# RchalYang/torchrl

Hardware: NVIDIA H100
Metric: env_steps_per_sec (higher is better)
Workload: dtype f32

## Files before the change

### include/torchrl_b200.h

```cpp
#ifndef TORCHRL_B200_H
#define TORCHRL_B200_H
#include <stdint.h>

#ifdef __cplusplus
extern "C" {
#endif

#define TRL_OK 0
#define TRL_EINVAL (-1)
#define TRL_EALIGN (-2)
#define TRL_EUNSUPPORTED (-3)

const char* trl_last_error(void);
int trl_abi_version(void);
int trl_device_info(int* sm_count, int* cc_major, int* cc_minor);

int trl_gae_scan(const float* rewards, const float* values, const uint8_t* terminals,
                 const uint8_t* time_limits, const float* last_value, float* advs, float* returns,
                 int64_t T, int64_t N, float gamma, float tau, int time_limit_filter, int variant,
                 void* stream);

int trl_discount_return(const float* rewards, const float* values, const uint8_t* terminals,
                        const uint8_t* time_limits, const float* last_value, float* advs, float* returns,
                        int64_t T, int64_t N, float gamma, int time_limit_filter, int variant,
                        void* stream);

int trl_synth_env_smem_bytes(int obs_dim, int act_dim);
int trl_synth_env_num_ctas(int64_t N);
int trl_synth_env_step(float* state, const float* actions, const float* A, const float* B, const float* c,
                       const float* lb, const float* ub, int* elapsed, const int* step_count, float* reward,
                       uint8_t* done, uint8_t* time_limit, double* partial, double* batch_sums,
                       double* norm_mean, double* norm_var, double* norm_count, unsigned* ticket,
                       int* any_reset, const int* t_ptr, int64_t N, int obs_dim, int act_dim, float rho,
                       float eta, float ctrl_cost, float term_thr, float reward_scale, int max_episode_steps,
                       int max_episode_frames, int merge_stats, void* stream);
int trl_synth_env_reset(float* state, int* elapsed, unsigned* episode, const unsigned* seeds,
                        const uint8_t* mask, int64_t N, int obs_dim, double init_scale, void* stream);
int trl_synth_env_seed(unsigned* seeds, unsigned* episode, int64_t N, unsigned seed, unsigned n_total,
                       unsigned first_env, void* stream);

int trl_obs_norm_moments(const float* x, int64_t N, int obs_dim, double* sums, void* stream);
int trl_obs_norm_merge(const double* sums, double batch_n, int obs_dim, double* mean, double* var,
                       double* count, void* stream);
int trl_obs_norm_filt(const float* raw, const double* mean, const double* var, int64_t N, int obs_dim,
                      double clip, float* out, void* stream);

int trl_tanh_gaussian_sample(const float* mean, const float* log_std, int ls_stride, const float* eps,
                             float noise_scale, uint64_t seed, const uint64_t* rng_counter, int64_t M,
                             int act_dim, int tanh_action, float* action, float* pre_tanh, float* log_prob,
                             float* eps_out, int* nan_flag, void* stream);
int trl_tanh_gaussian_sample_bwd(const float* action, const float* eps, const float* log_std, int ls_stride,
                                 const float* g_action, const float* g_logp, int64_t M, int act_dim,
                                 int tanh_action, float* g_mean, float* g_log_std, void* stream);

int trl_collect_finalize(const float* cur_ob_in, const float* next_norm, float* state, const float* act,
                         const float* value, const float* v_next, const float* reward, const uint8_t* done,
                         const uint8_t* tl, int* elapsed, unsigned* episode, const unsigned* seeds,
                         int* step_count, double* ep_return, double* epoch_reward, float* ret_log,
                         int* n_done, const int* any_reset, const double* norm_mean, const double* norm_var,
                         float* cur_ob_out, float* b_obs, float* b_next_obs, float* b_acts, float* b_values,
                         float* b_rewards, uint8_t* b_terminals, uint8_t* b_time_limits, const int* t_ptr,
                         int64_t N, int obs_dim, int act_dim, int max_episode_frames, float discount,
                         double init_scale, double clip, int terminal_includes_surpass,
                         int raw_obs_after_reset, void* stream);
int trl_step_advance(int* t_ptr, int T, int* size_ptr, uint64_t* rng_counter, void* stream);

int trl_row_gather(int nkeys, const void* const* src, void* const* dst, const int64_t* row_bytes,
                   const int64_t* idx, const int* pos_ptr, int rows, void* stream);
int trl_ring_write(int nkeys, const void* const* src, void* const* dst, const int64_t* row_bytes,
                   const int* row_ptr, void* stream);
int trl_ring_write_advance(int nkeys, const void* const* src, void* const* dst, const int64_t* row_bytes,
                           int* row_ptr, int T, int* size_ptr, unsigned* ticket, void* stream);
int trl_vec_stats(const float* x, int64_t n, float* stats4, void* stream);
int trl_vec_moments(const float* x, int64_t n, double* moments4, void* stream);
int trl_row_group_moments(const float* x, const int64_t* idx, int groups, int b, int64_t row_elems,
                          double* moments4, void* stream);
int trl_group_stats_from_moments(const double* gathered, int world, int groups, double n_total, float* stats4,
                                 void* stream);
int trl_vec_stats_from_moments(const double* gathered, int world, double n_total, float* stats4, void* stream);

int64_t trl_ppo_actor_scratch_doubles(int64_t B, int act_dim);
int trl_ppo_actor_loss(const float* mean, const float* log_std, int ls_stride, const float* actions,
                       const float* old_logp, const float* advs, const float* adv_stats,
                       const int* adv_stats_pos ,
                       int64_t B,
                       int act_dim, int tanh_action, float clip_para, float entropy_coeff, float ls_min, float ls_max,
                       float* g_mean, float* g_log_std, float* logp_out, float* info16, double* scratch, unsigned* ticket,
                       void* stream);
int trl_ppo_critic_loss(const float* values, const float* returns, const float* old_values, int64_t B,
                        int clipped, float clip_para, float* g_values, float* info1, double* scratch,
                        unsigned* ticket, void* stream);
int trl_gaussian_log_prob(const float* mean, const float* log_std, int ls_stride, const float* actions,
                          int64_t B, int act_dim, int tanh_action, float* logp, void* stream);

int trl_categorical_sample(const float* logits, const float* u, uint64_t seed, const uint64_t* rng_counter, int64_t M,
                           int num_actions, float* action, float* log_prob, int* nan_flag, void* stream);
int trl_categorical_log_prob(const float* logits, const float* actions, int64_t M, int num_actions, float* logp,
                             void* stream);
int64_t trl_ppo_categorical_actor_scratch_doubles(int64_t B);
int trl_ppo_categorical_actor_loss(const float* logits, const float* actions, const float* old_logp, const float* advs,
                                   const float* adv_stats, const int* adv_stats_pos, int64_t B, int num_actions,
                                   float clip_para, float entropy_coeff, float* g_logits, float* logp_out,
                                   float* info16, double* scratch, unsigned* ticket, void* stream);

int trl_grad_sumsq_blocks(int nseg);
int trl_grad_sumsq(const float* grad, const int64_t* seg_begin_host, int nseg, unsigned active_mask,
                   double* sumsq3_out, int* step_counts, double beta1, double beta2, double* scratch,
                   unsigned* ticket, void* stream);
int trl_adam_step(float* param, float* grad, float* exp_avg, float* exp_avg_sq, const int64_t* seg_begin_host,
                  int nseg, unsigned active_mask, const double* sumsq3, const float* lr_dev,
                  const float* max_norm_host, const float* eps_host, float beta1, float beta2,
                  float grad_scale, int zero_grad, float* param_hi, float* param_lo, void* stream);
int trl_polyak_update(float* target, const float* source, int64_t n, float tau, float* target_hi,
                      float* target_lo, void* stream);

int64_t trl_offpolicy_scratch_doubles(int64_t B);
int trl_td_target(const float* rewards, const uint8_t* terminals, const float* q1_next, const float* q2_next,
                  const float* logp_next, const float* log_alpha, float fixed_alpha, float gamma, int64_t B,
                  float* y, float* info1, double* scratch, unsigned* ticket, void* stream);
int trl_td3_smooth_action(const float* action, const float* eps, float sigma, float noise_clip, uint64_t seed,
                          const uint64_t* rng_counter, int64_t n, float* out, void* stream);
int trl_sac_alpha_step(const float* logp, float target_entropy, float* log_alpha, float* adam_state3, float lr,
                       float beta1, float beta2, float eps, int64_t B, float* info2, double* scratch,
                       unsigned* ticket, void* stream);
int trl_sac_policy_loss(const float* logp, const float* q1, const float* q2, const float* log_alpha,
                        float fixed_alpha, int64_t B, float* g_logp, float* g_q1, float* g_q2, float* info5,
                        double* scratch, unsigned* ticket, void* stream);
int trl_twin_mse_loss(const float* q1, const float* q2, const float* y, int64_t B, float* g1, float* g2,
                      float* info2, double* scratch, unsigned* ticket, void* stream);
int trl_qr_dqn_loss(const float* pred, const float* next, const float* actions, const float* rewards,
                    const uint8_t* terminals, const float* weights, int B, int n_actions, int n_quantiles,
                    float gamma, float kappa, int mse, float* grad, float* td_out, float* info3, double* scratch,
                    unsigned* ticket, void* stream);

int64_t trl_bias_act_bwd_scratch_floats(int64_t M, int H);
int trl_bias_act_fwd(float* z, const float* bias, int64_t M, int H, int act, void* stream);
int trl_bias_act_bwd(const float* grad, const float* out, float* grad_pre, float* dbias, int64_t M, int H,
                     int act, float* scratch, unsigned* tickets, void* stream);
int trl_split_tf32(const float* x, int64_t n, float* hi, float* lo, void* stream);

int trl_per_sample(const float* prio, int size, const double* u, int b, float beta, int64_t* idx,
                   float* weights, void* stream);
int trl_per_update(float* prio, const int64_t* idx, const float* td, int b, int n, float alpha, float eps,
                   float* max_prio, void* stream);
int trl_per_insert(float* prio, const int* row_ptr, const float* max_prio, void* stream);

int trl_frame_ring_write(const uint8_t* stack, uint8_t* ring, uint8_t* age_ring, const int* elapsed, uint8_t* hist,
                         int* hist_count, const int* top, const int* size, int64_t N, int C, int64_t F, int T, int frame,
                         void* stream);
int trl_frame_hist_advance(int* hist_count, const int* size, int T, void* stream);
int trl_frame_stack_gather(const uint8_t* obs_last, const uint8_t* next_last, const uint8_t* age, const uint8_t* hist,
                           const int* hist_count, const int64_t* idx, const int* pos, int rows, const int* top,
                           const int* size, int64_t N, int C, int64_t F, int T, float scale, float* out_obs,
                           float* out_next, void* stream);

int trl_comm_flag_bytes(void);
int trl_comm_ipc_handle_bytes(void);
int trl_comm_alloc(int64_t bytes, void** ptr_out);
int trl_comm_free(void* ptr);
int trl_comm_ipc_get(void* ptr, void* handle_out);
int trl_comm_ipc_open(const void* handle, void** ptr_out);
int trl_comm_ipc_close(void* ptr);
int trl_comm_scratch_doubles(int nseg);
int trl_allreduce_grad(const void* const* peer_data, void* const* peer_flags, int rank, int world, float* out,
                       int64_t n, const int64_t* seg_begin_host, int nseg, unsigned active_mask, double* sumsq3_out,
                       int* step_counts, double beta1, double beta2, double* scratch, unsigned* ticket, unsigned* seq,
                       int zero_local, void* stream);
int trl_allreduce_f64(const void* const* peer_data, void* const* peer_flags, int rank, int world, double* out, int n,
                      int gather, unsigned* seq, void* stream);
int64_t trl_comm_ll_recv_bytes(int world, int nmax);
int trl_allreduce_f64_ll(const double* local, void* const* peer_recv, int rank, int world, double* out, int n, int nmax,
                         int gather, unsigned* ll_seq, void* stream);

int trl_gemm_tf32x3_nt(const float* A, const float* B, float* C, int64_t M, int64_t K, int splits,
                       float* workspace, const float* bias, int act, void* stream);
int trl_gemm_tf32x3_tn(const float* A, const float* B, float* C, int64_t M, int64_t K, int splits,
                       float* workspace, void* stream);
int trl_transpose_f32(const float* in, float* out, int64_t rows, int cols, void* stream);
int trl_gemm3_pair(const float* A, const float* b_hi, const float* b_lo, float* C, int64_t M, int64_t K,
                   int b_nmajor, const float* bias, int act, void* stream);
int trl_gemm3_pair_tn(const float* A, const float* B, float* C, int64_t M, int64_t K, int splits,
                      float* workspace, void* stream);
int trl_gemm3_pair_tn_cluster(const float* A, const float* B, float* C, int64_t M, int64_t K, int splits,
                              float* workspace, int* tickets, void* stream);

int trl_skinny_k_fwd(const float* X, const float* W, const float* bias, float* Y, int64_t M, int K, int H,
                     int act, void* stream);
int64_t trl_skinny_tn_scratch_floats(int64_t M, int H, int K);
int trl_skinny_tn(const float* A, const float* B, float* Out, float* colsum, int64_t M, int H, int K,
                  int out_transposed, float* scratch, void* stream);
int trl_skinny_n_fwd(const float* X, const float* W, const float* bias, float* Y, int64_t M, int H, int N,
                     void* stream);
int trl_skinny_n_dgrad(const float* G, const float* W, float* dX, int64_t M, int H, int N, void* stream);
int trl_skinny_act_wgrad(const float* G, const float* Y, const float* X, float* dW, float* db, int64_t M, int H,
                         int K, int act, float* scratch, void* stream);
int64_t trl_skinny_dgrad_act_scratch_floats(int64_t M, int H);
int trl_skinny_n_dgrad_act(const float* G, const float* W, const float* Y, float* gz, float* db, int64_t M, int H,
                           int N, int act, float* scratch, void* stream);
int trl_skinny_tn_partial(const float* A, const float* B, int64_t M, int H, int K, int want_colsum, float* scratch,
                          void* stream);
int trl_skinny_act_wgrad_partial(const float* G, const float* Y, const float* X, int64_t M, int H, int K, int act,
                                 float* scratch, void* stream);
int trl_skinny_n_dgrad_act_partial(const float* G, const float* W, const float* Y, float* gz, int64_t M, int H, int N,
                                   int act, float* scratch, void* stream);
int trl_skinny_reduce_jobs(int njobs, const int* kind, const float* const* scratch, float* const* out,
                           float* const* colsum, const int64_t* M, const int* H, const int* K, const int* out_transposed,
                           void* stream);

int trl_synth_atari_step(uint8_t* obs, int* latent, const float* actions, int* elapsed, float* reward,
                         uint8_t* done, uint8_t* time_limit, int64_t N, int max_steps, void* stream);
int trl_synth_atari_reset(uint8_t* obs, int* latent, int* elapsed, unsigned* episode, const unsigned* seeds,
                          const uint8_t* mask, const int* zero_is_mask, int episode_bias, int bump, int64_t N,
                          void* stream);
int trl_u8_to_f32(const uint8_t* in, float* out, int64_t n, float scale, void* stream);

#ifdef __cplusplus
}
#endif
#endif
```

### torchrl_b200/_lib.py

```python
import ctypes
import os

_HERE = os.path.dirname(os.path.abspath(__file__))
LIB_PATH = os.path.join(_HERE, "lib", "libtorchrl_b200.so")

c_f32p = ctypes.c_void_p
c_u8p = ctypes.c_void_p
c_i32p = ctypes.c_void_p
c_i64p = ctypes.c_void_p
c_f64p = ctypes.c_void_p
vp = ctypes.c_void_p
i64 = ctypes.c_int64
i32 = ctypes.c_int
f32 = ctypes.c_float
f64 = ctypes.c_double
u64 = ctypes.c_uint64
u32 = ctypes.c_uint32

SIGNATURES = {
    "trl_last_error": [],
    "trl_abi_version": [],
    "trl_device_info": [vp, vp, vp],
    "trl_gae_scan": [vp, vp, vp, vp, vp, vp, vp, i64, i64, f32, f32, i32, i32, vp],
    "trl_discount_return": [vp, vp, vp, vp, vp, vp, vp, i64, i64, f32, i32, i32, vp],
    "trl_synth_env_smem_bytes": [i32, i32],
    "trl_synth_env_num_ctas": [i64],
    "trl_synth_env_step": [vp] * 20 + [i64, i32, i32, f32, f32, f32, f32, f32, i32, i32, i32, vp],
    "trl_synth_env_reset": [vp, vp, vp, vp, vp, i64, i32, f64, vp],
    "trl_synth_env_seed": [vp, vp, i64, u32, u32, u32, vp],
    "trl_obs_norm_moments": [vp, i64, i32, vp, vp],
    "trl_obs_norm_merge": [vp, f64, i32, vp, vp, vp, vp],
    "trl_obs_norm_filt": [vp, vp, vp, i64, i32, f64, vp, vp],
    "trl_tanh_gaussian_sample": [vp, vp, i32, vp, f32, u64, vp, i64, i32, i32, vp, vp, vp, vp, vp, vp],
    "trl_tanh_gaussian_sample_bwd": [vp, vp, vp, i32, vp, vp, i64, i32, i32, vp, vp, vp],
    "trl_collect_finalize": [vp] * 29 + [i64, i32, i32, i32, f32, f64, f64, i32, i32, vp],
    "trl_step_advance": [vp, i32, vp, vp, vp],
    "trl_row_gather": [i32, vp, vp, vp, vp, vp, i32, vp],
    "trl_ring_write": [i32, vp, vp, vp, vp, vp],
    "trl_ring_write_advance": [i32, vp, vp, vp, vp, i32, vp, vp, vp],
    "trl_vec_stats": [vp, i64, vp, vp],
    "trl_vec_moments": [vp, i64, vp, vp],
    "trl_vec_stats_from_moments": [vp, i32, f64, vp, vp],
    "trl_row_group_moments": [vp, vp, i32, i32, i64, vp, vp],
    "trl_group_stats_from_moments": [vp, i32, i32, f64, vp, vp],
    "trl_ppo_actor_scratch_doubles": [i64, i32],
    "trl_ppo_actor_loss": [vp, vp, i32, vp, vp, vp, vp, vp, i64, i32, i32, f32, f32, f32, f32, vp, vp, vp, vp, vp, vp, vp],
    "trl_ppo_critic_loss": [vp, vp, vp, i64, i32, f32, vp, vp, vp, vp, vp],
    "trl_gaussian_log_prob": [vp, vp, i32, vp, i64, i32, i32, vp, vp],
    "trl_categorical_sample": [vp, vp, u64, vp, i64, i32, vp, vp, vp, vp],
    "trl_categorical_log_prob": [vp, vp, i64, i32, vp, vp],
    "trl_ppo_categorical_actor_scratch_doubles": [i64],
    "trl_ppo_categorical_actor_loss": [vp, vp, vp, vp, vp, vp, i64, i32, f32, f32, vp, vp, vp, vp, vp, vp],
    "trl_grad_sumsq_blocks": [i32],
    "trl_grad_sumsq": [vp, vp, i32, u32, vp, vp, f64, f64, vp, vp, vp],
    "trl_adam_step": [vp, vp, vp, vp, vp, i32, u32, vp, vp, vp, vp, f32, f32, f32, i32, vp, vp, vp],
    "trl_polyak_update": [vp, vp, i64, f32, vp, vp, vp],
    "trl_bias_act_bwd_scratch_floats": [i64, i32],
    "trl_bias_act_fwd": [vp, vp, i64, i32, i32, vp],
    "trl_split_tf32": [vp, i64, vp, vp, vp],
    "trl_bias_act_bwd": [vp, vp, vp, vp, i64, i32, i32, vp, vp, vp],
    "trl_per_sample": [vp, i32, vp, i32, f32, vp, vp, vp],
    "trl_per_update": [vp, vp, vp, i32, i32, f32, f32, vp, vp],
    "trl_per_insert": [vp, vp, vp, vp],
    "trl_gemm_tf32x3_nt": [vp, vp, vp, i64, i64, i32, vp, vp, i32, vp],
    "trl_gemm_tf32x3_tn": [vp, vp, vp, i64, i64, i32, vp, vp],
    "trl_transpose_f32": [vp, vp, i64, i32, vp],
    "trl_frame_ring_write": [vp, vp, vp, vp, vp, vp, vp, vp, i64, i32, i64, i32, i32, vp],
    "trl_frame_hist_advance": [vp, vp, i32, vp],
    "trl_frame_stack_gather": [vp, vp, vp, vp, vp, vp, vp, i32, vp, vp, i64, i32, i64, i32, f32, vp, vp, vp],
    "trl_comm_flag_bytes": [],
    "trl_comm_ipc_handle_bytes": [],
    "trl_comm_alloc": [i64, vp],
    "trl_comm_free": [vp],
    "trl_comm_ipc_get": [vp, vp],
    "trl_comm_ipc_open": [vp, vp],
    "trl_comm_ipc_close": [vp],
    "trl_comm_scratch_doubles": [i32],
    "trl_allreduce_grad": [vp, vp, i32, i32, vp, i64, vp, i32, u32, vp, vp, f64, f64, vp, vp, vp, i32, vp],
    "trl_allreduce_f64": [vp, vp, i32, i32, vp, i32, i32, vp, vp],
    "trl_comm_ll_recv_bytes": [i32, i32],
    "trl_allreduce_f64_ll": [vp, vp, i32, i32, vp, i32, i32, i32, vp, vp],
    "trl_gemm3_pair": [vp, vp, vp, vp, i64, i64, i32, vp, i32, vp],
    "trl_gemm3_pair_tn": [vp, vp, vp, i64, i64, i32, vp, vp],
    "trl_gemm3_pair_tn_cluster": [vp, vp, vp, i64, i64, i32, vp, vp, vp],
    "trl_skinny_k_fwd": [vp, vp, vp, vp, i64, i32, i32, i32, vp],
    "trl_skinny_tn_scratch_floats": [i64, i32, i32],
    "trl_skinny_tn": [vp, vp, vp, vp, i64, i32, i32, i32, vp, vp],
    "trl_skinny_n_fwd": [vp, vp, vp, vp, i64, i32, i32, vp],
    "trl_skinny_n_dgrad": [vp, vp, vp, i64, i32, i32, vp],
    "trl_skinny_act_wgrad": [vp, vp, vp, vp, vp, i64, i32, i32, i32, vp, vp],
    "trl_skinny_dgrad_act_scratch_floats": [i64, i32],
    "trl_skinny_n_dgrad_act": [vp, vp, vp, vp, vp, i64, i32, i32, i32, vp, vp],
    "trl_skinny_tn_partial": [vp, vp, i64, i32, i32, i32, vp, vp],
    "trl_skinny_act_wgrad_partial": [vp, vp, vp, i64, i32, i32, i32, vp, vp],
    "trl_skinny_n_dgrad_act_partial": [vp, vp, vp, vp, i64, i32, i32, i32, vp, vp],
    "trl_skinny_reduce_jobs": [i32, vp, vp, vp, vp, vp, vp, vp, vp, vp],
    "trl_synth_atari_step": [vp, vp, vp, vp, vp, vp, vp, i64, i32, vp],
    "trl_synth_atari_reset": [vp, vp, vp, vp, vp, vp, vp, i32, i32, i64, vp],
    "trl_u8_to_f32": [vp, vp, i64, f32, vp],
    "trl_offpolicy_scratch_doubles": [i64],
    "trl_td_target": [vp, vp, vp, vp, vp, vp, f32, f32, i64, vp, vp, vp, vp, vp],
    "trl_td3_smooth_action": [vp, vp, f32, f32, u64, vp, i64, vp, vp],
    "trl_sac_alpha_step": [vp, f32, vp, vp, f32, f32, f32, f32, i64, vp, vp, vp, vp],
    "trl_sac_policy_loss": [vp, vp, vp, vp, f32, i64, vp, vp, vp, vp, vp, vp, vp],
    "trl_twin_mse_loss": [vp, vp, vp, i64, vp, vp, vp, vp, vp, vp],
    "trl_qr_dqn_loss": [vp, vp, vp, vp, vp, vp, i32, i32, i32, f32, f32, i32, vp, vp, vp, vp, vp, vp],
}
_RESTYPES = {"trl_last_error": ctypes.c_char_p, "trl_ppo_actor_scratch_doubles": ctypes.c_int64,
             "trl_ppo_categorical_actor_scratch_doubles": ctypes.c_int64,
             "trl_offpolicy_scratch_doubles": ctypes.c_int64, "trl_bias_act_bwd_scratch_floats": ctypes.c_int64,
             "trl_skinny_tn_scratch_floats": ctypes.c_int64,
             "trl_skinny_dgrad_act_scratch_floats": ctypes.c_int64, "trl_comm_ll_recv_bytes": ctypes.c_int64}
_VALUE_FUNCS = ("trl_abi_version", "trl_synth_env_smem_bytes", "trl_synth_env_num_ctas", "trl_comm_flag_bytes",
                "trl_comm_ipc_handle_bytes", "trl_comm_scratch_doubles", "trl_comm_ll_recv_bytes",
                "trl_ppo_actor_scratch_doubles", "trl_ppo_categorical_actor_scratch_doubles", "trl_grad_sumsq_blocks")

_lib = None


class NativeLibraryError(RuntimeError):
    pass


def load():
    global _lib
    if _lib is not None:
        return _lib
    if not os.path.exists(LIB_PATH) and os.environ.get("TORCHRL_B200_NO_AUTOBUILD") != "1":
        try:
            from . import build as _build
            _build.build()
        except Exception as e:
            raise NativeLibraryError("%s not found and the in-tree nvcc build failed (%s); there is no CPU "
                                     "fallback" % (LIB_PATH, e)) from e
    if not os.path.exists(LIB_PATH):
        raise NativeLibraryError(
            "%s not found: build it with `python -m torchrl_b200.build` (there is no CPU fallback)" % LIB_PATH)
    lib = ctypes.CDLL(LIB_PATH)
    for name, argtypes in SIGNATURES.items():
        try:
            fn = getattr(lib, name)
        except AttributeError as e:
            raise NativeLibraryError("symbol %s missing from %s" % (name, LIB_PATH)) from e
        fn.argtypes = argtypes
        fn.restype = _RESTYPES.get(name, ctypes.c_int)
    _lib = lib
    return lib


def check(rc, name):
    if rc != 0:
        msg = load().trl_last_error()
        raise RuntimeError("%s failed (rc=%d): %s" % (name, rc, msg.decode() if msg else ""))


_LAUNCHES = 0


def launch_count():
    return _LAUNCHES


def add_launches(n):
    global _LAUNCHES
    _LAUNCHES += int(n)


def call(name, *args):
    global _LAUNCHES
    lib = load()
    rc = getattr(lib, name)(*args)
    if rc != 0:
        check(rc, name)
    _LAUNCHES += 1
```

### torchrl_b200/csrc/gemm_wgmma.cuh

```cuda
#pragma once
#include "common.cuh"
#include "reduce.cuh"
#include <cuda.h>

namespace trl {
namespace wg {

constexpr int kBM = 128, kBN = 128, kN = 256, kBK = 32;
constexpr int kTileBytes = 128 * kBK * 4;
constexpr int kConsumers = 256;
constexpr int kThreads = kConsumers + 128;
constexpr int kProducerRegs = 40, kConsumerRegs = 232;

template <bool BMN, bool BSPLIT>
struct Ring {
  static constexpr int kTiles = 3 + (BMN ? (BSPLIT ? 2 : 1) : 0);
  static constexpr int kStageBytes = kTiles * kTileBytes;
  static constexpr int kStages = (200 * 1024) / kStageBytes < 4 ? (200 * 1024) / kStageBytes : 4;
  static constexpr int kSmemBytes = kStages * kStageBytes + 1024  + 128 ;
  static constexpr bool kConvertB = BMN || !BSPLIT;
  static_assert(kStages >= 2 && kSmemBytes <= 227 * 1024, "fits one sm_90 CTA");
};

__device__ __forceinline__ uint32_t smem_u32(const void* p) { return static_cast<uint32_t>(__cvta_generic_to_shared(p)); }
__device__ __forceinline__ void mbar_init(uint64_t* bar, uint32_t count) {
  asm volatile("mbarrier.init.shared::cta.b64 [%0], %1;" ::"r"(smem_u32(bar)), "r"(count));
}
__device__ __forceinline__ void mbar_arrive(uint64_t* bar) {
  asm volatile("mbarrier.arrive.shared::cta.b64 _, [%0];" ::"r"(smem_u32(bar)) : "memory");
}
__device__ __forceinline__ void mbar_arrive_expect_tx(uint64_t* bar, uint32_t bytes) {
  asm volatile("mbarrier.arrive.expect_tx.shared::cta.b64 _, [%0], %1;" ::"r"(smem_u32(bar)), "r"(bytes) : "memory");
}
__device__ __forceinline__ void mbar_wait(uint64_t* bar, uint32_t parity) {
  uint32_t done;
  do {
    asm volatile(
        "{\n\t"
        ".reg .pred p;\n\t"
        "mbarrier.try_wait.parity.shared::cta.b64 p, [%1], %2;\n\t"
        "selp.u32 %0, 1, 0, p;\n\t"
        "}"
        : "=r"(done)
        : "r"(smem_u32(bar)), "r"(parity)
        : "memory");
  } while (!done);
}
__device__ __forceinline__ void tma_load_2d(void* smem_dst, const CUtensorMap* map, uint64_t* bar, int c_inner, int c_outer) {
  asm volatile(
      "cp.async.bulk.tensor.2d.shared::cluster.global.mbarrier::complete_tx::bytes [%0], [%1, {%3, %4}], [%2];" ::"r"(
          smem_u32(smem_dst)),
      "l"(reinterpret_cast<uint64_t>(map)), "r"(smem_u32(bar)), "r"(c_inner), "r"(c_outer)
      : "memory");
}

__device__ __forceinline__ uint64_t desc_k_sw128(uint32_t smem_addr) {
  uint64_t d = 0;
  d |= static_cast<uint64_t>((smem_addr >> 4) & 0x3FFF);
  d |= static_cast<uint64_t>(1) << 16;
  d |= static_cast<uint64_t>(1024 >> 4) << 32;
  d |= static_cast<uint64_t>(1) << 62;
  return d;
}

__device__ __forceinline__ void wgmma_m64n128k8_tf32_rs(float (&d)[64], const uint32_t (&a)[4], uint64_t desc_b) {
  asm volatile(
      "{\n\t"
      ".reg .pred p;\n\t"
      "setp.ne.b32 p, %69, 0;\n\t"
      "wgmma.mma_async.sync.aligned.m64n128k8.f32.tf32.tf32 "
      "{%0, %1, %2, %3, %4, %5, %6, %7, %8, %9, %10, %11, %12, %13, %14, %15, "
      "%16, %17, %18, %19, %20, %21, %22, %23, %24, %25, %26, %27, %28, %29, %30, %31, "
      "%32, %33, %34, %35, %36, %37, %38, %39, %40, %41, %42, %43, %44, %45, %46, %47, "
      "%48, %49, %50, %51, %52, %53, %54, %55, %56, %57, %58, %59, %60, %61, %62, %63}, "
      "{%64, %65, %66, %67}, %68, p, 1, 1;\n\t"
      "}"
      : "+f"(d[0]), "+f"(d[1]), "+f"(d[2]), "+f"(d[3]), "+f"(d[4]), "+f"(d[5]), "+f"(d[6]), "+f"(d[7]),
        "+f"(d[8]), "+f"(d[9]), "+f"(d[10]), "+f"(d[11]), "+f"(d[12]), "+f"(d[13]), "+f"(d[14]), "+f"(d[15]),
        "+f"(d[16]), "+f"(d[17]), "+f"(d[18]), "+f"(d[19]), "+f"(d[20]), "+f"(d[21]), "+f"(d[22]), "+f"(d[23]),
        "+f"(d[24]), "+f"(d[25]), "+f"(d[26]), "+f"(d[27]), "+f"(d[28]), "+f"(d[29]), "+f"(d[30]), "+f"(d[31]),
        "+f"(d[32]), "+f"(d[33]), "+f"(d[34]), "+f"(d[35]), "+f"(d[36]), "+f"(d[37]), "+f"(d[38]), "+f"(d[39]),
        "+f"(d[40]), "+f"(d[41]), "+f"(d[42]), "+f"(d[43]), "+f"(d[44]), "+f"(d[45]), "+f"(d[46]), "+f"(d[47]),
        "+f"(d[48]), "+f"(d[49]), "+f"(d[50]), "+f"(d[51]), "+f"(d[52]), "+f"(d[53]), "+f"(d[54]), "+f"(d[55]),
        "+f"(d[56]), "+f"(d[57]), "+f"(d[58]), "+f"(d[59]), "+f"(d[60]), "+f"(d[61]), "+f"(d[62]), "+f"(d[63])
      : "r"(a[0]), "r"(a[1]), "r"(a[2]), "r"(a[3]), "l"(desc_b), "r"(1));
}

__device__ __forceinline__ float4 lds128(uint32_t addr) {
  float4 v;
  asm volatile("ld.shared.v4.f32 {%0, %1, %2, %3}, [%4];" : "=f"(v.x), "=f"(v.y), "=f"(v.z), "=f"(v.w) : "r"(addr));
  return v;
}
__device__ __forceinline__ float lds32(uint32_t addr) {
  float v;
  asm volatile("ld.shared.f32 %0, [%1];" : "=f"(v) : "r"(addr));
  return v;
}
__device__ __forceinline__ void sts128(uint32_t addr, const float4 v) {
  asm volatile("st.shared.v4.f32 [%0], {%1, %2, %3, %4};" ::"r"(addr), "f"(v.x), "f"(v.y), "f"(v.z), "f"(v.w));
}
__device__ __forceinline__ uint32_t cluster_rank() {
  uint32_t r;
  asm volatile("mov.u32 %0, %%cluster_ctarank;" : "=r"(r));
  return r;
}
__device__ __forceinline__ uint32_t cluster_size() {
  uint32_t n;
  asm volatile("mov.u32 %0, %%cluster_nctarank;" : "=r"(n));
  return n;
}
__device__ __forceinline__ void cluster_arrive() { asm volatile("barrier.cluster.arrive.release;" ::: "memory"); }
__device__ __forceinline__ void cluster_wait() { asm volatile("barrier.cluster.wait.acquire;" ::: "memory"); }
__device__ __forceinline__ float4 ld_cluster128(uint32_t addr, uint32_t rank) {
  uint32_t remote;
  asm volatile("mapa.shared::cluster.u32 %0, %1, %2;" : "=r"(remote) : "r"(addr), "r"(rank));
  float4 v;
  asm volatile("ld.shared::cluster.v4.f32 {%0, %1, %2, %3}, [%4];"
               : "=f"(v.x), "=f"(v.y), "=f"(v.z), "=f"(v.w)
               : "r"(remote)
               : "memory");
  return v;
}
__device__ __forceinline__ uint32_t tf32_bits(float x) {
  uint32_t u;
  asm("cvt.rna.tf32.f32 %0, %1;" : "=r"(u) : "f"(x));
  return u;
}
__device__ __forceinline__ float4 tf32_hi(const float4 v) {
  return make_float4(__uint_as_float(tf32_bits(v.x)), __uint_as_float(tf32_bits(v.y)), __uint_as_float(tf32_bits(v.z)),
                     __uint_as_float(tf32_bits(v.w)));
}
__device__ __forceinline__ float4 sub4(const float4 a, const float4 b) {
  return make_float4(a.x - b.x, a.y - b.y, a.z - b.z, a.w - b.w);
}

__device__ __forceinline__ float4 load_unit_mn(uint32_t raw, int u, int& row, int& chunk) {
  row = u & 127; chunk = u >> 7;
  const uint32_t a = raw + static_cast<uint32_t>(chunk * 4 * 128 + row) * 4u;
  return make_float4(lds32(a), lds32(a + 512u), lds32(a + 1024u), lds32(a + 1536u));
}
__device__ __forceinline__ uint32_t sw128(int row, int chunk) {
  return static_cast<uint32_t>(row * 128 + ((chunk ^ (row & 7)) << 4));
}

template <bool AMN>
__device__ __forceinline__ uint32_t a_offset(int m, int k) {
  if (!AMN) return static_cast<uint32_t>(m * 128 + ((((k >> 2) ^ (m & 7))) << 4) + (k & 3) * 4);
  return static_cast<uint32_t>((m >> 5) * 4096 + k * 128 + ((((m & 31) >> 2) ^ (k & 7)) << 4) + (m & 3) * 4);
}

struct Params {
  const float* __restrict__ bias;
  int act;
  float* __restrict__ C;
  long long M;
  int k_blocks_per_split;
  float* __restrict__ ws;
  unsigned* tickets;
};

constexpr int kTileLd = kBN + 8;

template <bool AMN, bool BMN, bool BSPLIT, bool TANH_MUFU, bool CLUSTER = false>
__global__ void __launch_bounds__(kThreads, 1)
gemm3_wgmma_kernel(const __grid_constant__ CUtensorMap map_a, const __grid_constant__ CUtensorMap map_b,
                   const __grid_constant__ CUtensorMap map_b2, const Params p) {
  using R = Ring<BMN, BSPLIT>;
  constexpr int S = R::kStages;
  constexpr int kA = 0, kBhi = kTileBytes, kBlo = 2 * kTileBytes, kBraw = 3 * kTileBytes, kBraw2 = 4 * kTileBytes;
  extern __shared__ uint8_t smem_raw[];
  uint8_t* ring = reinterpret_cast<uint8_t*>((reinterpret_cast<uintptr_t>(smem_raw) + 1023) & ~static_cast<uintptr_t>(1023));
  uint64_t* bars = reinterpret_cast<uint64_t*>(ring + S * R::kStageBytes);
  uint64_t* full = bars;
  uint64_t* empty = bars + S;
  uint64_t* conv = bars + 2 * S;

  const int warp = threadIdx.x >> 5, lane = threadIdx.x & 31;
  const int m_blk = blockIdx.x, n0 = blockIdx.y * kBN;
  const int c_size = CLUSTER ? static_cast<int>(cluster_size()) : 1, c_rank = CLUSTER ? static_cast<int>(cluster_rank()) : 0;
  const int split = CLUSTER ? static_cast<int>(blockIdx.z) / c_size + 8 * c_rank : static_cast<int>(blockIdx.z);
  const int nkb = p.k_blocks_per_split;
  const int kb0 = split * nkb;

  if (threadIdx.x == kConsumers) {
    asm volatile("prefetch.tensormap [%0];" ::"l"(reinterpret_cast<uint64_t>(&map_a)) : "memory");
    asm volatile("prefetch.tensormap [%0];" ::"l"(reinterpret_cast<uint64_t>(&map_b)) : "memory");
    if (BSPLIT) asm volatile("prefetch.tensormap [%0];" ::"l"(reinterpret_cast<uint64_t>(&map_b2)) : "memory");
    for (int s = 0; s < S; ++s) {
      mbar_init(&full[s], 1);
      mbar_init(&empty[s], kConsumers / 32);
      mbar_init(&conv[s], kConsumers / 32);
    }
    asm volatile("fence.mbarrier_init.release.cluster;" ::: "memory");
  }
  __syncthreads();

  if (warp >= kConsumers / 32) {
    asm volatile("setmaxnreg.dec.sync.aligned.u32 %0;" ::"n"(kProducerRegs));
    if (warp == kConsumers / 32 && lane == 0) {
      for (int kb = 0; kb < nkb; ++kb) {
        const int s = kb % S;
        const uint32_t ph = (kb / S) & 1;
        mbar_wait(&empty[s], ph ^ 1);
        uint8_t* st = ring + s * R::kStageBytes;
        mbar_arrive_expect_tx(&full[s], (BSPLIT ? 3 : 2) * kTileBytes);
        const int k0 = (kb0 + kb) * kBK;
        if (AMN) {
#pragma unroll
          for (int j = 0; j < 4; ++j) tma_load_2d(st + kA + j * 4096, &map_a, &full[s], m_blk * kBM + 32 * j, k0);
        } else {
          tma_load_2d(st + kA, &map_a, &full[s], k0, m_blk * kBM);
        }
        if (BMN) {
          tma_load_2d(st + kBraw, &map_b, &full[s], n0, k0);
          if (BSPLIT) tma_load_2d(st + kBraw2, &map_b2, &full[s], n0, k0);
        } else {
          tma_load_2d(st + kBhi, &map_b, &full[s], k0, n0);
          if (BSPLIT) tma_load_2d(st + kBlo, &map_b2, &full[s], k0, n0);
        }
      }
    }
    if constexpr (CLUSTER) {
      __syncwarp();
      __syncthreads();
      cluster_arrive();
      cluster_wait();
      cluster_arrive();
      last_cta(p.tickets + (m_blk * 2 + blockIdx.y) * 8 + c_rank, 8u);
      cluster_wait();
    }
    return;
  }

  asm volatile("setmaxnreg.inc.sync.aligned.u32 %0;" ::"n"(kConsumerRegs));
  const int ct = threadIdx.x, wgi = warp >> 2, wl = warp & 3;
  const int gid = lane >> 2, tid = lane & 3;
  const int am = wgi * 64 + wl * 16 + gid;
  float acc[64], cor[64];
#pragma unroll
  for (int i = 0; i < 64; ++i) { acc[i] = 0.f; cor[i] = 0.f; }
  for (int kb = 0; kb < nkb; ++kb) {
    const int s = kb % S;
    const uint32_t ph = (kb / S) & 1;
    const uint32_t st = smem_u32(ring + s * R::kStageBytes);
    mbar_wait(&full[s], ph);
    if (R::kConvertB) {
      float4 vb[4], vl[4];
      int rb[4], cb[4];
      if (BMN) {
#pragma unroll
        for (int i = 0; i < 4; ++i) vb[i] = load_unit_mn(st + kBraw, ct + i * kConsumers, rb[i], cb[i]);
        if (BSPLIT) {
#pragma unroll
          for (int i = 0; i < 4; ++i) vl[i] = load_unit_mn(st + kBraw2, ct + i * kConsumers, rb[i], cb[i]);
        }
      } else {
#pragma unroll
        for (int i = 0; i < 4; ++i) vb[i] = lds128(st + kBhi + static_cast<uint32_t>(ct + i * kConsumers) * 16u);
      }
#pragma unroll
      for (int i = 0; i < 4; ++i) {
        const uint32_t o = BMN ? sw128(rb[i], cb[i]) : static_cast<uint32_t>(ct + i * kConsumers) * 16u;
        if (BSPLIT) {
          sts128(st + kBhi + o, vb[i]);
          sts128(st + kBlo + o, vl[i]);
        } else {
          const float4 h = tf32_hi(vb[i]);
          sts128(st + kBhi + o, h);
          sts128(st + kBlo + o, sub4(vb[i], h));
        }
      }
      asm volatile("fence.proxy.async.shared::cta;" ::: "memory");
      __syncwarp();
      if (lane == 0) mbar_arrive(&conv[s]);
    }
    uint32_t ahi[kBK / 8][4], alo[kBK / 8][4];
    {
      float av[kBK / 8][4];
#pragma unroll
      for (int k = 0; k < kBK / 8; ++k)
#pragma unroll
        for (int r = 0; r < 4; ++r) av[k][r] = lds32(st + kA + a_offset<AMN>(am + 8 * (r & 1), 8 * k + tid + 4 * (r >> 1)));
#pragma unroll
      for (int k = 0; k < kBK / 8; ++k)
#pragma unroll
        for (int r = 0; r < 4; ++r) {
          ahi[k][r] = tf32_bits(av[k][r]);
          alo[k][r] = __float_as_uint(av[k][r] - __uint_as_float(ahi[k][r]));
        }
    }
    if (R::kConvertB) mbar_wait(&conv[s], ph);
    const uint64_t db_hi = desc_k_sw128(st + kBhi), db_lo = desc_k_sw128(st + kBlo);
    asm volatile("wgmma.fence.sync.aligned;" ::: "memory");
#pragma unroll
    for (int k = 0; k < kBK / 8; ++k) {
      const uint64_t adv = static_cast<uint64_t>((k * 8 * 4) >> 4);
      wgmma_m64n128k8_tf32_rs(cor, alo[k], db_hi + adv);
      wgmma_m64n128k8_tf32_rs(cor, ahi[k], db_lo + adv);
      wgmma_m64n128k8_tf32_rs(acc, ahi[k], db_hi + adv);
    }
    asm volatile("wgmma.commit_group.sync.aligned;" ::: "memory");
    asm volatile("wgmma.wait_group.sync.aligned 0;" ::: "memory");
    __syncwarp();
    if (lane == 0) mbar_arrive(&empty[s]);
  }

  if constexpr (CLUSTER) {
    __syncthreads();
    float* tile = reinterpret_cast<float*>(ring);
#pragma unroll
    for (int j = 0; j < 16; ++j)
#pragma unroll
      for (int h = 0; h < 2; ++h)
        *reinterpret_cast<float2*>(tile + (am + 8 * h) * kTileLd + j * 8 + 2 * tid) =
            make_float2(acc[4 * j + 2 * h] + cor[4 * j + 2 * h], acc[4 * j + 2 * h + 1] + cor[4 * j + 2 * h + 1]);
    cluster_arrive();
    cluster_wait();
    const int r_lo = c_rank * kBM / c_size, n_vec = ((c_rank + 1) * kBM / c_size - r_lo) * (kBN / 4);
    const long long slab = p.M * kN;
    const uint32_t tile_u32 = smem_u32(tile);
    for (int v = ct; v < n_vec; v += kConsumers) {
      const int r = r_lo + v / (kBN / 4), q4 = v % (kBN / 4);
      const uint32_t a = tile_u32 + static_cast<uint32_t>(r * kTileLd + 4 * q4) * 4u;
      float4 x[8];
#pragma unroll
      for (int q = 0; q < 8; ++q)
        if (q < c_size) x[q] = ld_cluster128(a, static_cast<uint32_t>(q));
      float4 s = make_float4(0.f, 0.f, 0.f, 0.f);
#pragma unroll
      for (int q = 0; q < 8; ++q)
        if (q < c_size) { s.x += x[q].x; s.y += x[q].y; s.z += x[q].z; s.w += x[q].w; }
      const long long o = (static_cast<long long>(m_blk) * kBM + r) * kN + n0 + 4 * q4;
      *reinterpret_cast<float4*>(p.ws + (static_cast<long long>(blockIdx.z) / c_size) * slab + o) = s;
    }
    cluster_arrive();
    if (last_cta(p.tickets + (m_blk * 2 + blockIdx.y) * 8 + c_rank, 8u)) {
      for (int v = ct; v < n_vec; v += kConsumers) {
        const long long o = (static_cast<long long>(m_blk) * kBM + r_lo + v / (kBN / 4)) * kN + n0 + 4 * (v % (kBN / 4));
        float4 t[8];
#pragma unroll
        for (int g = 0; g < 8; ++g) t[g] = __ldcg(reinterpret_cast<const float4*>(p.ws + g * slab + o));
#define TRL_T3(c) (((t[0].c + t[1].c) + (t[2].c + t[3].c)) + ((t[4].c + t[5].c) + (t[6].c + t[7].c)))
        *reinterpret_cast<float4*>(p.C + o) = make_float4(TRL_T3(x), TRL_T3(y), TRL_T3(z), TRL_T3(w));
#undef TRL_T3
      }
    }
    cluster_wait();
    return;
  }
  const long long r0 = static_cast<long long>(m_blk) * kBM + am;
  float* cbase = p.C + static_cast<long long>(split) * p.M * kN;
  const bool has_bias = p.bias != nullptr;
#pragma unroll
  for (int j = 0; j < 16; ++j) {
    const int col = n0 + j * 8 + 2 * (lane & 3);
    float2 b = make_float2(0.f, 0.f);
    if (has_bias) b = __ldg(reinterpret_cast<const float2*>(p.bias + col));
#pragma unroll
    for (int h = 0; h < 2; ++h) {
      const long long row = r0 + 8 * h;
      float2 v = make_float2(acc[4 * j + 2 * h] + cor[4 * j + 2 * h], acc[4 * j + 2 * h + 1] + cor[4 * j + 2 * h + 1]);
      if (has_bias) {
        v.x += b.x; v.y += b.y;
        if (p.act == 1) {
          if (TANH_MUFU) { v.x = tanh_ex2(v.x); v.y = tanh_ex2(v.y); }
          else { v.x = tanhf(v.x); v.y = tanhf(v.y); }
        } else if (p.act == 2) {
          v.x = fmaxf(v.x, 0.f); v.y = fmaxf(v.y, 0.f);
        }
      }
      if (row < p.M) *reinterpret_cast<float2*>(cbase + row * kN + col) = v;
    }
  }
}

typedef CUresult (*PFN_encodeTiled)(CUtensorMap*, CUtensorMapDataType, cuuint32_t, void*, const cuuint64_t*,
                                    const cuuint64_t*, const cuuint32_t*, const cuuint32_t*, CUtensorMapInterleave,
                                    CUtensorMapSwizzle, CUtensorMapL2promotion, CUtensorMapFloatOOBfill);

inline PFN_encodeTiled get_encode() {
  static PFN_encodeTiled fn = nullptr;
  if (!fn) {
    void* ptr = nullptr;
    cudaDriverEntryPointQueryResult qres;
    if (cudaGetDriverEntryPoint("cuTensorMapEncodeTiled", &ptr, cudaEnableDefault, &qres) == cudaSuccess &&
        qres == cudaDriverEntryPointSuccess)
      fn = reinterpret_cast<PFN_encodeTiled>(ptr);
  }
  return fn;
}

enum class Box { kKMajor, kMNMajor, kMNMajorA };

inline bool make_map(CUtensorMap* map, const float* base, uint64_t rows, uint64_t cols, Box box_kind) {
  PFN_encodeTiled enc = get_encode();
  if (!enc) return false;
  const cuuint64_t gdim[2] = {cols, rows};
  const cuuint64_t gstride[1] = {cols * sizeof(float)};
  const cuuint32_t inner = box_kind == Box::kMNMajor ? 128 : kBK;
  const cuuint32_t box[2] = {inner, static_cast<cuuint32_t>(box_kind == Box::kKMajor ? 128 : kBK)};
  const cuuint32_t estr[2] = {1, 1};
  return enc(map, CU_TENSOR_MAP_DATA_TYPE_FLOAT32, 2, const_cast<float*>(base), gdim, gstride, box, estr,
             CU_TENSOR_MAP_INTERLEAVE_NONE,
             box_kind == Box::kMNMajor ? CU_TENSOR_MAP_SWIZZLE_NONE : CU_TENSOR_MAP_SWIZZLE_128B,
             CU_TENSOR_MAP_L2_PROMOTION_L2_256B, CU_TENSOR_MAP_FLOAT_OOB_FILL_NONE) == CUDA_SUCCESS;
}

template <bool AMN, bool BMN, bool BSPLIT, bool TANH_MUFU, bool CLUSTER = false>
int launch(const CUtensorMap& ma, const CUtensorMap& mb, const CUtensorMap& mb2, const Params& p, unsigned splits,
           cudaStream_t st, const char* what) {
  constexpr int kSmem = Ring<BMN, BSPLIT>::kSmemBytes;
  auto kernel = gemm3_wgmma_kernel<AMN, BMN, BSPLIT, TANH_MUFU, CLUSTER>;
  static bool attr_set = false;
  if (!attr_set) {
    cudaError_t e = cudaFuncSetAttribute(kernel, cudaFuncAttributeMaxDynamicSharedMemorySize, kSmem);
    if (e != cudaSuccess) { set_error("cudaFuncSetAttribute: %s", cudaGetErrorString(e)); return static_cast<int>(e); }
    attr_set = true;
  }
  const dim3 grid(static_cast<unsigned>(ceil_div<long long>(p.M, kBM)), kN / kBN, splits);
  if constexpr (CLUSTER) {
    cudaLaunchConfig_t cfg = {};
    cfg.gridDim = grid;
    cfg.blockDim = dim3(kThreads);
    cfg.dynamicSmemBytes = kSmem;
    cfg.stream = st;
    cudaLaunchAttribute attr[1];
    attr[0].id = cudaLaunchAttributeClusterDimension;
    attr[0].val.clusterDim.x = 1;
    attr[0].val.clusterDim.y = 1;
    attr[0].val.clusterDim.z = splits / 8;
    cfg.attrs = attr;
    cfg.numAttrs = 1;
    const cudaError_t e = cudaLaunchKernelEx(&cfg, kernel, ma, mb, mb2, p);
    if (e != cudaSuccess) { set_error("%s: %s", what, cudaGetErrorString(e)); return static_cast<int>(e); }
  } else {
    kernel<<<grid, kThreads, kSmem, st>>>(ma, mb, mb2, p);
  }
  return check_launch(what);
}

}
}
```

### torchrl_b200/csrc/skinny.cu

```cuda
#include "common.cuh"

namespace trl {

constexpr int kSkMaxRows = 128;
constexpr int kSkCtas = 2 * kNumSM;

__device__ __forceinline__ float sk_tanh(float x) { return tanh_ex2(x); }

__device__ __forceinline__ float4 sk_act4(float4 v, int act) {
  if (act == 1) return make_float4(sk_tanh(v.x), sk_tanh(v.y), sk_tanh(v.z), sk_tanh(v.w));
  if (act == 2) return make_float4(fmaxf(v.x, 0.f), fmaxf(v.y, 0.f), fmaxf(v.z, 0.f), fmaxf(v.w, 0.f));
  return v;
}

__device__ __forceinline__ float4 sk_dact4(float4 g, float4 y, int act) {
  if (act == 1)
    return make_float4(g.x * fmaf(-y.x, y.x, 1.f), g.y * fmaf(-y.y, y.y, 1.f), g.z * fmaf(-y.z, y.z, 1.f),
                       g.w * fmaf(-y.w, y.w, 1.f));
  if (act == 2) return make_float4(y.x > 0.f ? g.x : 0.f, y.y > 0.f ? g.y : 0.f, y.z > 0.f ? g.z : 0.f, y.w > 0.f ? g.w : 0.f);
  return g;
}

static inline int sk_rows_per_cta(long long M) {
  long long r = ceil_div<long long>(M, kSkCtas);
  if (r < 8) r = 8;
  if (r > kSkMaxRows) r = kSkMaxRows;
  return static_cast<int>(r);
}

template <int K>
__device__ __forceinline__ void stage_rows(float* __restrict__ dst, const float* __restrict__ src, long long row0,
                                           int nrows, int tid, int nthr) {
  constexpr int KP = (K + 3) & ~3;
  const float* base = src + row0 * K;
  for (int j = tid; j < nrows * K; j += nthr) {
    const int r = j / K, k = j - r * K;
    dst[r * KP + k] = __ldg(base + j);
  }
  if (KP != K) {
    constexpr int PAD = KP - K > 0 ? KP - K : 1;
    for (int j = tid; j < nrows * PAD; j += nthr) {
      const int r = j / PAD, k = K + (j - r * PAD);
      dst[r * KP + k] = 0.f;
    }
  }
}

template <int KP>
__device__ __forceinline__ void stage_rows_rt(float* __restrict__ dst, const float* __restrict__ src, long long row0,
                                              int nrows, int K, int tid, int nthr) {
  for (int i = tid; i < nrows * KP; i += nthr) {
    const int r = i / KP, k = i - r * KP;
    dst[i] = (k < K) ? __ldg(src + (row0 + r) * K + k) : 0.f;
  }
}

#define TRL_SK_FMA4(ACC, S, WK)                                                          \
  ACC.x = fmaf(S, WK[0], ACC.x); ACC.y = fmaf(S, WK[1], ACC.y);                          \
  ACC.z = fmaf(S, WK[2], ACC.z); ACC.w = fmaf(S, WK[3], ACC.w)

template <int K>
__global__ void __launch_bounds__(256, 2) skinny_k_fwd_kernel(const float* __restrict__ X, const float* __restrict__ W,
                                                             const float* __restrict__ bias, float* __restrict__ Y,
                                                             long long M, int H, int act, int rows_per_cta) {
  constexpr int KP = (K + 3) & ~3;
  extern __shared__ __align__(16) float sk_smem[];
  const int tid = threadIdx.x;
  const long long row0 = static_cast<long long>(blockIdx.x) * rows_per_cta;
  if (row0 >= M) return;
  const int nrows = static_cast<int>(min(static_cast<long long>(rows_per_cta), M - row0));
  const int HS = H + 4;
  float* wt = sk_smem + rows_per_cta * KP;
  {
    int h = tid / K, k = tid - h * K;
    constexpr int dh = 256 / K, dk = 256 % K;
    for (int i = tid; i < H * K; i += 256) {
      wt[k * HS + h] = __ldg(W + i);
      h += dh; k += dk;
      if (k >= K) { k -= K; ++h; }
    }
  }
  stage_rows<K>(sk_smem, X, row0, nrows, tid, 256);
  const int cpg = H >> 2;
  const int RL = 256 / cpg;
  const bool active = tid < RL * cpg;
  const int cg = tid % cpg, rl = tid / cpg;
  __syncthreads();
  if (!active) return;
  float w[KP][4];
#pragma unroll
  for (int k = 0; k < K; ++k) {
    const float4 v = *reinterpret_cast<const float4*>(wt + k * HS + 4 * cg);
    w[k][0] = v.x; w[k][1] = v.y; w[k][2] = v.z; w[k][3] = v.w;
  }
  const float4 bb = *reinterpret_cast<const float4*>(bias + 4 * cg);
  float* yp = Y + (row0 + rl) * H + 4 * cg;
  const long long ystep = static_cast<long long>(RL) * H;
  for (int r = rl; r < nrows; r += RL, yp += ystep) {
    const float4* xr = reinterpret_cast<const float4*>(sk_smem + r * KP);
    float4 acc = bb;
#pragma unroll
    for (int q = 0; q < KP / 4; ++q) {
      const float4 xv = xr[q];
      if (4 * q < K) { TRL_SK_FMA4(acc, xv.x, w[4 * q]); }
      if (4 * q + 1 < K) { TRL_SK_FMA4(acc, xv.y, w[4 * q + 1]); }
      if (4 * q + 2 < K) { TRL_SK_FMA4(acc, xv.z, w[4 * q + 2]); }
      if (4 * q + 3 < K) { TRL_SK_FMA4(acc, xv.w, w[4 * q + 3]); }
    }
    *reinterpret_cast<float4*>(yp) = sk_act4(acc, act);
  }
}

template <int K>
__device__ __forceinline__ void tn_fma_row(float (&acc)[(K + 3) & ~3][4], const float4 a, const float* __restrict__ brow) {
  constexpr int KP = (K + 3) & ~3;
  const float av[4] = {a.x, a.y, a.z, a.w};
#pragma unroll
  for (int q = 0; q < KP / 4; ++q) {
    const float4 b = reinterpret_cast<const float4*>(brow)[q];
#pragma unroll
    for (int j = 0; j < 4; ++j) {
      if (4 * q < K) acc[4 * q][j] = fmaf(av[j], b.x, acc[4 * q][j]);
      if (4 * q + 1 < K) acc[4 * q + 1][j] = fmaf(av[j], b.y, acc[4 * q + 1][j]);
      if (4 * q + 2 < K) acc[4 * q + 2][j] = fmaf(av[j], b.z, acc[4 * q + 2][j]);
      if (4 * q + 3 < K) acc[4 * q + 3][j] = fmaf(av[j], b.w, acc[4 * q + 3][j]);
    }
  }
}

template <int K, bool ACT>
__global__ void __launch_bounds__(256, 2) skinny_tn_kernel(const float* __restrict__ A, const float* __restrict__ Yact,
                                                          const float* __restrict__ B, int want_colsum, int act,
                                                          float* __restrict__ partial, long long M, int H,
                                                          int rows_per_cta) {
  constexpr int KP = (K + 3) & ~3;
  constexpr int U = ACT ? (K <= 17 ? 4 : (K <= 19 ? 2 : 1)) : (K <= 12 ? 8 : (K <= 17 ? 4 : 2));
  extern __shared__ __align__(16) float sk_smem[];
  const int tid = threadIdx.x, nthr = blockDim.x;
  const long long row0 = static_cast<long long>(blockIdx.x) * rows_per_cta;
  const int nrows = static_cast<int>(min(static_cast<long long>(rows_per_cta), M - row0));
  stage_rows<K>(sk_smem, B, row0, nrows, tid, nthr);
  __syncthreads();
  const int lane = tid & 31, warp = tid >> 5;
  const int cg = lane & 7, rl = lane >> 3;
  const int c0 = warp * 32 + cg * 4;
  float acc[KP][4];
#pragma unroll
  for (int k = 0; k < KP; ++k)
#pragma unroll
    for (int j = 0; j < 4; ++j) acc[k][j] = 0.f;
  float4 asum = make_float4(0.f, 0.f, 0.f, 0.f);
  const float* ap = A + row0 * H + c0;
  const float* yp = ACT ? Yact + row0 * H + c0 : nullptr;
  int r = rl;
  for (; r + 4 * (U - 1) < nrows; r += 4 * U) {
    float4 g[U], y[U];
#pragma unroll
    for (int u = 0; u < U; ++u) {
      g[u] = __ldg(reinterpret_cast<const float4*>(ap + static_cast<long long>(r + 4 * u) * H));
      if (ACT) y[u] = __ldg(reinterpret_cast<const float4*>(yp + static_cast<long long>(r + 4 * u) * H));
    }
#pragma unroll
    for (int u = 0; u < U; ++u) {
      float4 a0 = g[u];
      if (ACT) {
        a0 = sk_dact4(a0, y[u], act);
        asum.x += a0.x; asum.y += a0.y; asum.z += a0.z; asum.w += a0.w;
      }
      tn_fma_row<K>(acc, a0, sk_smem + (r + 4 * u) * KP);
    }
  }
  for (; r < nrows; r += 4) {
    float4 a0 = __ldg(reinterpret_cast<const float4*>(ap + static_cast<long long>(r) * H));
    if (ACT) {
      a0 = sk_dact4(a0, __ldg(reinterpret_cast<const float4*>(yp + static_cast<long long>(r) * H)), act);
      asum.x += a0.x; asum.y += a0.y; asum.z += a0.z; asum.w += a0.w;
    }
    tn_fma_row<K>(acc, a0, sk_smem + r * KP);
  }
#pragma unroll
  for (int k = 0; k < K; ++k)
#pragma unroll
    for (int j = 0; j < 4; ++j) {
      float v = acc[k][j];
      v += __shfl_xor_sync(0xffffffffu, v, 8);
      v += __shfl_xor_sync(0xffffffffu, v, 16);
      acc[k][j] = v;
    }
  float* pp = partial + static_cast<long long>(blockIdx.x) * (K + 1) * H;
#pragma unroll
  for (int k = 0; k < K; ++k) {
    if ((k & 3) == rl)
      *reinterpret_cast<float4*>(pp + static_cast<long long>(k) * H + c0) =
          make_float4(acc[k][0], acc[k][1], acc[k][2], acc[k][3]);
  }
  if (ACT) {
    asum.x += __shfl_xor_sync(0xffffffffu, asum.x, 8); asum.x += __shfl_xor_sync(0xffffffffu, asum.x, 16);
    asum.y += __shfl_xor_sync(0xffffffffu, asum.y, 8); asum.y += __shfl_xor_sync(0xffffffffu, asum.y, 16);
    asum.z += __shfl_xor_sync(0xffffffffu, asum.z, 8); asum.z += __shfl_xor_sync(0xffffffffu, asum.z, 16);
    asum.w += __shfl_xor_sync(0xffffffffu, asum.w, 8); asum.w += __shfl_xor_sync(0xffffffffu, asum.w, 16);
    if (rl == (K & 3)) *reinterpret_cast<float4*>(pp + static_cast<long long>(K) * H + c0) = asum;
  } else if (tid < K) {
    float s = 0.f;
    if (want_colsum)
      for (int rr = 0; rr < nrows; ++rr) s += sk_smem[rr * KP + tid];
    pp[static_cast<long long>(K) * H + tid] = s;
  }
}

constexpr int kRedGroups = 32;
constexpr int kRedElems = 8;
__device__ __forceinline__ void tn_reduce_block(const float* __restrict__ partial, float* __restrict__ Out,
                                                float* __restrict__ colsum, int n_cs, int nslab, int H, int K,
                                                int out_transposed, int block, float (*red)[kRedElems + 1]) {
  const int el = threadIdx.x & (kRedElems - 1), g = threadIdx.x / kRedElems;
  const int e = block * kRedElems + el;
  const int n_main = K * H;
  const int n_all = n_main + n_cs;
  const long long stride = static_cast<long long>(K + 1) * H;
  float s0 = 0.f, s1 = 0.f, s2 = 0.f, s3 = 0.f;
  if (e < n_all) {
    const float* pe = partial + e;
    int sl = g;
    for (; sl + 3 * kRedGroups < nslab; sl += 4 * kRedGroups) {
      const float v0 = __ldcg(pe + static_cast<long long>(sl) * stride);
      const float v1 = __ldcg(pe + static_cast<long long>(sl + kRedGroups) * stride);
      const float v2 = __ldcg(pe + static_cast<long long>(sl + 2 * kRedGroups) * stride);
      const float v3 = __ldcg(pe + static_cast<long long>(sl + 3 * kRedGroups) * stride);
      s0 += v0; s1 += v1; s2 += v2; s3 += v3;
    }
    for (; sl < nslab; sl += kRedGroups) s0 += __ldcg(pe + static_cast<long long>(sl) * stride);
  }
  red[g][el] = (s0 + s1) + (s2 + s3);
  __syncthreads();
  if (g == 0 && e < n_all) {
    float s = red[0][el];
#pragma unroll
    for (int i = 1; i < kRedGroups; ++i) s += red[i][el];
    if (e < n_main) {
      const int k = e / H, h = e - k * H;
      if (out_transposed) Out[e] = s;
      else Out[static_cast<long long>(h) * K + k] = s;
    } else {
      colsum[e - n_main] = s;
    }
  }
}

__global__ void __launch_bounds__(kRedElems * kRedGroups) skinny_tn_reduce_kernel(const float* __restrict__ partial,
                                                                                 float* __restrict__ Out,
                                                                                 float* __restrict__ colsum, int n_cs,
                                                                                 int nslab, int H, int K,
                                                                                 int out_transposed) {
  __shared__ float red[kRedGroups][kRedElems + 1];
  tn_reduce_block(partial, Out, colsum, n_cs, nslab, H, K, out_transposed, blockIdx.x, red);
}

constexpr int kMaxRedJobs = 8;
struct ReduceJobs {
  const float* partial[kMaxRedJobs];
  float* out[kMaxRedJobs];
  float* colsum[kMaxRedJobs];
  int n_cs[kMaxRedJobs], nslab[kMaxRedJobs], H[kMaxRedJobs], K[kMaxRedJobs], out_t[kMaxRedJobs];
  int cta_begin[kMaxRedJobs + 1];
  int njobs;
};
__global__ void __launch_bounds__(kRedElems * kRedGroups) skinny_reduce_jobs_kernel(const ReduceJobs q) {
  __shared__ float red[kRedGroups][kRedElems + 1];
  int j = 0;
#pragma unroll
  for (int i = 1; i < kMaxRedJobs; ++i) j += (i < q.njobs && static_cast<int>(blockIdx.x) >= q.cta_begin[i]) ? 1 : 0;
  tn_reduce_block(q.partial[j], q.out[j], q.colsum[j], q.n_cs[j], q.nslab[j], q.H[j], q.K[j], q.out_t[j],
                  static_cast<int>(blockIdx.x) - q.cta_begin[j], red);
}

template <int NB>
__device__ __forceinline__ float nb_butterfly(float (&v)[NB], int lane) {
  int off = 16;
#pragma unroll
  for (int cnt = NB; cnt > 1; cnt >>= 1) {
    const int half = cnt >> 1;
    const bool hi = lane & off;
#pragma unroll
    for (int i = 0; i < half; ++i) {
      const float send = hi ? v[i] : v[i + half];
      const float keep = hi ? v[i + half] : v[i];
      v[i] = keep + __shfl_xor_sync(0xffffffffu, send, off);
    }
    off >>= 1;
  }
  for (; off > 0; off >>= 1) v[0] += __shfl_xor_sync(0xffffffffu, v[0], off);
  return v[0];
}
template <int NB>
__device__ __forceinline__ int nb_out_index(int lane) {
  int n = 0, off = 16;
#pragma unroll
  for (int cnt = NB; cnt > 1; cnt >>= 1) {
    if (lane & off) n += cnt >> 1;
    off >>= 1;
  }
  return n;
}

template <int HC, int NB>
__global__ void __launch_bounds__(256, 2) skinny_n_fwd_kernel(const float* __restrict__ X, const float* __restrict__ W,
                                                             const float* __restrict__ bias, float* __restrict__ Y,
                                                             long long M, int H, int N) {
  const int lane = threadIdx.x & 31;
  const long long gw = static_cast<long long>(blockIdx.x) * 8 + (threadIdx.x >> 5);
  const long long nw = static_cast<long long>(gridDim.x) * 8;
  float4 w[NB][HC];
#pragma unroll
  for (int n = 0; n < NB; ++n)
#pragma unroll
    for (int c = 0; c < HC; ++c)
      w[n][c] = (n < N) ? *reinterpret_cast<const float4*>(W + static_cast<long long>(n) * H + c * 128 + lane * 4)
                        : make_float4(0.f, 0.f, 0.f, 0.f);
  const int n_out = nb_out_index<NB>(lane);
  const bool writer = (lane & (32 / NB - 1)) == 0 && n_out < N;
  const float b_out = (n_out < N) ? bias[n_out] : 0.f;
  constexpr int R = (NB == 8 && HC == 2) ? 3 : 4;
  for (long long m0 = gw * R; m0 < M; m0 += nw * R) {
    float4 x[R][HC];
#pragma unroll
    for (int i = 0; i < R; ++i)
#pragma unroll
      for (int c = 0; c < HC; ++c)
        x[i][c] = (m0 + i < M) ? __ldg(reinterpret_cast<const float4*>(X + (m0 + i) * H + c * 128 + lane * 4))
                               : make_float4(0.f, 0.f, 0.f, 0.f);
#pragma unroll
    for (int i = 0; i < R; ++i) {
      float v[NB];
#pragma unroll
      for (int n = 0; n < NB; ++n) {
        float s = 0.f;
#pragma unroll
        for (int c = 0; c < HC; ++c)
          s = fmaf(x[i][c].x, w[n][c].x, fmaf(x[i][c].y, w[n][c].y, fmaf(x[i][c].z, w[n][c].z, fmaf(x[i][c].w, w[n][c].w, s))));
        v[n] = s;
      }
      const float tot = nb_butterfly<NB>(v, lane);
      if (writer && m0 + i < M) Y[(m0 + i) * N + n_out] = tot + b_out;
    }
  }
}

template <bool ACT>
__global__ void __launch_bounds__(256, 2) skinny_n_dgrad_kernel(const float* __restrict__ G, const float* __restrict__ W,
                                                               const float* __restrict__ Yact, int act,
                                                               float* __restrict__ dX, float* __restrict__ colpart,
                                                               long long M, int H, int N, int rows_per_cta) {
  extern __shared__ __align__(16) float sk_smem[];
  __shared__ __align__(16) float colred[1024];
  const int tid = threadIdx.x;
  const long long row0 = static_cast<long long>(blockIdx.x) * rows_per_cta;
  const int nrows = static_cast<int>(min(static_cast<long long>(rows_per_cta), M - row0));
  stage_rows_rt<8>(sk_smem, G, row0, nrows, N, tid, 256);
  const int cpg = H >> 2;
  const int RL = 256 / cpg;
  const bool active = tid < RL * cpg;
  const int cg = tid % cpg, rl = tid / cpg;
  float4 w[8];
#pragma unroll
  for (int n = 0; n < 8; ++n)
    w[n] = (active && n < N) ? *reinterpret_cast<const float4*>(W + static_cast<long long>(n) * H + 4 * cg)
                             : make_float4(0.f, 0.f, 0.f, 0.f);
  __syncthreads();
  float4 cs = make_float4(0.f, 0.f, 0.f, 0.f);
  auto row_out = [&](int r, float4 yv) {
    const float4 g0 = reinterpret_cast<const float4*>(sk_smem + r * 8)[0];
    const float4 g1 = reinterpret_cast<const float4*>(sk_smem + r * 8)[1];
    float4 acc;
    acc.x = g0.x * w[0].x; acc.y = g0.x * w[0].y; acc.z = g0.x * w[0].z; acc.w = g0.x * w[0].w;
    acc.x = fmaf(g0.y, w[1].x, acc.x); acc.y = fmaf(g0.y, w[1].y, acc.y); acc.z = fmaf(g0.y, w[1].z, acc.z); acc.w = fmaf(g0.y, w[1].w, acc.w);
    acc.x = fmaf(g0.z, w[2].x, acc.x); acc.y = fmaf(g0.z, w[2].y, acc.y); acc.z = fmaf(g0.z, w[2].z, acc.z); acc.w = fmaf(g0.z, w[2].w, acc.w);
    acc.x = fmaf(g0.w, w[3].x, acc.x); acc.y = fmaf(g0.w, w[3].y, acc.y); acc.z = fmaf(g0.w, w[3].z, acc.z); acc.w = fmaf(g0.w, w[3].w, acc.w);
    acc.x = fmaf(g1.x, w[4].x, acc.x); acc.y = fmaf(g1.x, w[4].y, acc.y); acc.z = fmaf(g1.x, w[4].z, acc.z); acc.w = fmaf(g1.x, w[4].w, acc.w);
    acc.x = fmaf(g1.y, w[5].x, acc.x); acc.y = fmaf(g1.y, w[5].y, acc.y); acc.z = fmaf(g1.y, w[5].z, acc.z); acc.w = fmaf(g1.y, w[5].w, acc.w);
    acc.x = fmaf(g1.z, w[6].x, acc.x); acc.y = fmaf(g1.z, w[6].y, acc.y); acc.z = fmaf(g1.z, w[6].z, acc.z); acc.w = fmaf(g1.z, w[6].w, acc.w);
    acc.x = fmaf(g1.w, w[7].x, acc.x); acc.y = fmaf(g1.w, w[7].y, acc.y); acc.z = fmaf(g1.w, w[7].z, acc.z); acc.w = fmaf(g1.w, w[7].w, acc.w);
    if (ACT) {
      acc = sk_dact4(acc, yv, act);
      cs.x += acc.x; cs.y += acc.y; cs.z += acc.z; cs.w += acc.w;
    }
    *reinterpret_cast<float4*>(dX + (row0 + r) * H + 4 * cg) = acc;
  };
  if (active) {
    const float4 z4 = make_float4(0.f, 0.f, 0.f, 0.f);
    int r = rl;
    if (ACT) {
      const float* yp = Yact + row0 * H + 4 * cg;
      for (; r + 3 * RL < nrows; r += 4 * RL) {
        const float4 y0 = __ldg(reinterpret_cast<const float4*>(yp + static_cast<long long>(r) * H));
        const float4 y1 = __ldg(reinterpret_cast<const float4*>(yp + static_cast<long long>(r + RL) * H));
        const float4 y2 = __ldg(reinterpret_cast<const float4*>(yp + static_cast<long long>(r + 2 * RL) * H));
        const float4 y3 = __ldg(reinterpret_cast<const float4*>(yp + static_cast<long long>(r + 3 * RL) * H));
        row_out(r, y0); row_out(r + RL, y1); row_out(r + 2 * RL, y2); row_out(r + 3 * RL, y3);
      }
      for (; r < nrows; r += RL) row_out(r, __ldg(reinterpret_cast<const float4*>(yp + static_cast<long long>(r) * H)));
    } else {
      for (; r < nrows; r += RL) row_out(r, z4);
    }
  }
  if (ACT) {
    if (active) *reinterpret_cast<float4*>(colred + rl * H + 4 * cg) = cs;
    __syncthreads();
    for (int c = tid; c < H; c += blockDim.x) {
      float s = colred[c];
      for (int i = 1; i < RL; ++i) s += colred[i * H + c];
      colpart[static_cast<long long>(blockIdx.x) * H + c] = s;
    }
  }
}

}

TRL_API int trl_skinny_k_fwd(const float* X, const float* W, const float* bias, float* Y, int64_t M, int K, int H,
                             int act, void* stream) {
  using namespace trl;
  TRL_REQUIRE(M >= 1 && K >= 1 && K <= 24 && H >= 4 && H % 4 == 0 && H <= 1024,
              "trl_skinny_k_fwd: need 1<=K<=24, H%%4==0, H<=1024 (K=%d H=%d)", K, H);
  TRL_REQUIRE(X && W && bias && Y, "trl_skinny_k_fwd: null pointer");
  TRL_REQUIRE(aligned16(bias) && aligned16(Y), "trl_skinny_k_fwd: bias/Y must be 16-byte aligned");
  const int rows = sk_rows_per_cta(M);
  const unsigned grid = static_cast<unsigned>(ceil_div<long long>(M, rows));
  cudaStream_t st = static_cast<cudaStream_t>(stream);
  const int kp = (K + 3) & ~3;
  const size_t smem = sizeof(float) * (static_cast<size_t>(rows) * kp + static_cast<size_t>(K) * (H + 4));
#define TRL_KF(KK)                                                                                                    \
  case KK: {                                                                                                          \
    if (smem > 48 * 1024) {                                                                                           \
      static bool raised = false;                                                                                     \
      if (!raised) {                                                                                                  \
        cudaError_t e = cudaFuncSetAttribute(skinny_k_fwd_kernel<KK>, cudaFuncAttributeMaxDynamicSharedMemorySize, 112 * 1024); \
        if (e != cudaSuccess) { set_error("cudaFuncSetAttribute: %s", cudaGetErrorString(e)); return static_cast<int>(e); } \
        raised = true;                                                                                                \
      }                                                                                                               \
    }                                                                                                                 \
    skinny_k_fwd_kernel<KK><<<grid, 256, smem, st>>>(X, W, bias, Y, M, H, act, rows);                                 \
  } break
  switch (K) {
    TRL_KF(1); TRL_KF(2); TRL_KF(3); TRL_KF(4); TRL_KF(5); TRL_KF(6); TRL_KF(7); TRL_KF(8);
    TRL_KF(9); TRL_KF(10); TRL_KF(11); TRL_KF(12); TRL_KF(13); TRL_KF(14); TRL_KF(15); TRL_KF(16);
    TRL_KF(17); TRL_KF(18); TRL_KF(19); TRL_KF(20); TRL_KF(21); TRL_KF(22); TRL_KF(23); TRL_KF(24);
  }
#undef TRL_KF
  return check_launch("skinny_k_fwd_kernel");
}

TRL_API int64_t trl_skinny_tn_scratch_floats(int64_t M, int H, int K) {
  const int rows = trl::sk_rows_per_cta(M);
  return trl::ceil_div<long long>(M, rows) * (K + 1) * H;
}

static int launch_skinny_tn(const float* A, const float* Yact, const float* B, float* Out, float* colsum, int64_t M,
                            int H, int K, int out_transposed, int act, bool fused_act, float* scratch, void* stream,
                            const char* who, bool defer = false) {
  using namespace trl;
  TRL_REQUIRE(M >= 1 && K >= 1 && K <= 24 && H >= 32 && H % 32 == 0 && H <= 256,
              "%s: need 1<=K<=24, H%%32==0, H<=256 (K=%d H=%d)", who, K, H);
  TRL_REQUIRE(A && B && Out && scratch, "%s: null pointer", who);
  TRL_REQUIRE(aligned16(A) && aligned16(scratch) && (!Yact || aligned16(Yact)), "%s: A/Y/scratch must be 16-byte aligned", who);
  const int rows = sk_rows_per_cta(M);
  const int nslab = static_cast<int>(ceil_div<long long>(M, rows));
  cudaStream_t st = static_cast<cudaStream_t>(stream);
  const int wc = colsum ? 1 : 0;
  const int kp = (K + 3) & ~3;
  const size_t smem = sizeof(float) * rows * kp;
  const unsigned nthr = static_cast<unsigned>(H);
#define TRL_TN(KK)                                                                                              \
  case KK:                                                                                                      \
    if (fused_act) skinny_tn_kernel<KK, true><<<nslab, nthr, smem, st>>>(A, Yact, B, wc, act, scratch, M, H, rows);   \
    else skinny_tn_kernel<KK, false><<<nslab, nthr, smem, st>>>(A, nullptr, B, wc, act, scratch, M, H, rows);   \
    break
  switch (K) {
    TRL_TN(1); TRL_TN(2); TRL_TN(3); TRL_TN(4); TRL_TN(5); TRL_TN(6); TRL_TN(7); TRL_TN(8);
    TRL_TN(9); TRL_TN(10); TRL_TN(11); TRL_TN(12); TRL_TN(13); TRL_TN(14); TRL_TN(15); TRL_TN(16);
    TRL_TN(17); TRL_TN(18); TRL_TN(19); TRL_TN(20); TRL_TN(21); TRL_TN(22); TRL_TN(23); TRL_TN(24);
  }
#undef TRL_TN
  int rc = check_launch("skinny_tn_kernel");
  if (rc != TRL_OK || defer) return rc;
  const int n_cs = colsum ? (fused_act ? H : K) : 0;
  const int n_all = K * H + n_cs;
  skinny_tn_reduce_kernel<<<ceil_div(n_all, kRedElems), kRedElems * kRedGroups, 0, st>>>(scratch, Out, colsum, n_cs, nslab, H, K, out_transposed);
  return check_launch("skinny_tn_reduce_kernel");
}

TRL_API int trl_skinny_tn(const float* A, const float* B, float* Out, float* colsum, int64_t M, int H, int K,
                          int out_transposed, float* scratch, void* stream) {
  return launch_skinny_tn(A, nullptr, B, Out, colsum, M, H, K, out_transposed, 0, false, scratch, stream, "trl_skinny_tn");
}

TRL_API int trl_skinny_act_wgrad(const float* G, const float* Y, const float* X, float* dW, float* db, int64_t M, int H,
                                 int K, int act, float* scratch, void* stream) {
  using namespace trl;
  TRL_REQUIRE(Y && db, "trl_skinny_act_wgrad: null pointer");
  TRL_REQUIRE(act >= 0 && act <= 2, "trl_skinny_act_wgrad: unknown activation %d", act);
  return launch_skinny_tn(G, Y, X, dW, db, M, H, K, 0, act, true, scratch, stream, "trl_skinny_act_wgrad");
}

TRL_API int trl_skinny_n_fwd(const float* X, const float* W, const float* bias, float* Y, int64_t M, int H, int N,
                             void* stream) {
  using namespace trl;
  TRL_REQUIRE(M >= 1 && N >= 1 && N <= 8 && (H == 128 || H == 256),
              "trl_skinny_n_fwd: need N<=8 and H in {128, 256} (N=%d H=%d)", N, H);
  TRL_REQUIRE(X && W && bias && Y, "trl_skinny_n_fwd: null pointer");
  TRL_REQUIRE(aligned16(X) && aligned16(W), "trl_skinny_n_fwd: X/W must be 16-byte aligned");
  long long blocks = ceil_div<long long>(M, 8 * 3);
  if (blocks > 2 * kNumSM) blocks = 2 * kNumSM;
  cudaStream_t st = static_cast<cudaStream_t>(stream);
  const unsigned grid = static_cast<unsigned>(blocks);
#define TRL_NF(HC, NB) skinny_n_fwd_kernel<HC, NB><<<grid, 256, 0, st>>>(X, W, bias, Y, M, H, N)
#define TRL_NF_H(HC)                  \
  do {                                \
    if (N == 1) TRL_NF(HC, 1);        \
    else if (N == 2) TRL_NF(HC, 2);   \
    else if (N <= 4) TRL_NF(HC, 4);   \
    else TRL_NF(HC, 8);               \
  } while (0)
  if (H == 128) TRL_NF_H(1);
  else TRL_NF_H(2);
#undef TRL_NF_H
#undef TRL_NF
  return check_launch("skinny_n_fwd_kernel");
}

TRL_API int trl_skinny_n_dgrad(const float* G, const float* W, float* dX, int64_t M, int H, int N, void* stream) {
  using namespace trl;
  TRL_REQUIRE(M >= 1 && N >= 1 && N <= 8 && H >= 4 && H % 4 == 0 && H <= 1024,
              "trl_skinny_n_dgrad: need N<=8, H%%4==0, H<=1024");
  TRL_REQUIRE(G && W && dX, "trl_skinny_n_dgrad: null pointer");
  TRL_REQUIRE(aligned16(W) && aligned16(dX), "trl_skinny_n_dgrad: W/dX must be 16-byte aligned");
  const int rows = sk_rows_per_cta(M);
  const unsigned grid = static_cast<unsigned>(ceil_div<long long>(M, rows));
  skinny_n_dgrad_kernel<false><<<grid, 256, sizeof(float) * rows * 8, static_cast<cudaStream_t>(stream)>>>(
      G, W, nullptr, 0, dX, nullptr, M, H, N, rows);
  return check_launch("skinny_n_dgrad_kernel");
}

TRL_API int64_t trl_skinny_dgrad_act_scratch_floats(int64_t M, int H) {
  return trl::ceil_div<long long>(M, trl::sk_rows_per_cta(M)) * H;
}

static int launch_n_dgrad_act(const float* G, const float* W, const float* Y, float* gz, float* db, int64_t M, int H, int N,
                              int act, float* scratch, void* stream, bool defer) {
  using namespace trl;
  TRL_REQUIRE(M >= 1 && N >= 1 && N <= 8 && H >= 4 && H % 4 == 0 && H <= 1024,
              "trl_skinny_n_dgrad_act: need N<=8, H%%4==0, H<=1024");
  TRL_REQUIRE(G && W && Y && gz && (db || defer) && scratch, "trl_skinny_n_dgrad_act: null pointer");
  TRL_REQUIRE(act >= 0 && act <= 2, "trl_skinny_n_dgrad_act: unknown activation %d", act);
  TRL_REQUIRE(aligned16(W) && aligned16(gz) && aligned16(Y), "trl_skinny_n_dgrad_act: W/Y/gz must be 16-byte aligned");
  const int rows = sk_rows_per_cta(M);
  const int nslab = static_cast<int>(ceil_div<long long>(M, rows));
  cudaStream_t st = static_cast<cudaStream_t>(stream);
  skinny_n_dgrad_kernel<true><<<nslab, 256, sizeof(float) * rows * 8, st>>>(G, W, Y, act, gz, scratch, M, H, N, rows);
  int rc = check_launch("skinny_n_dgrad_kernel");
  if (rc != TRL_OK || defer) return rc;
  skinny_tn_reduce_kernel<<<ceil_div(H, kRedElems), kRedElems * kRedGroups, 0, st>>>(scratch, db, db, H, nslab, H, 0, 0);
  return check_launch("skinny_tn_reduce_kernel");
}

TRL_API int trl_skinny_n_dgrad_act(const float* G, const float* W, const float* Y, float* gz, float* db, int64_t M,
                                   int H, int N, int act, float* scratch, void* stream) {
  return launch_n_dgrad_act(G, W, Y, gz, db, M, H, N, act, scratch, stream, false);
}

TRL_API int trl_skinny_tn_partial(const float* A, const float* B, int64_t M, int H, int K, int want_colsum, float* scratch,
                                  void* stream) {
  float dummy;
  return launch_skinny_tn(A, nullptr, B, &dummy, want_colsum ? &dummy : nullptr, M, H, K, 0, 0, false, scratch, stream,
                          "trl_skinny_tn_partial", true);
}

TRL_API int trl_skinny_act_wgrad_partial(const float* G, const float* Y, const float* X, int64_t M, int H, int K, int act,
                                         float* scratch, void* stream) {
  using namespace trl;
  TRL_REQUIRE(Y, "trl_skinny_act_wgrad_partial: null pointer");
  TRL_REQUIRE(act >= 0 && act <= 2, "trl_skinny_act_wgrad_partial: unknown activation %d", act);
  float dummy;
  return launch_skinny_tn(G, Y, X, &dummy, &dummy, M, H, K, 0, act, true, scratch, stream, "trl_skinny_act_wgrad_partial", true);
}

TRL_API int trl_skinny_n_dgrad_act_partial(const float* G, const float* W, const float* Y, float* gz, int64_t M, int H, int N,
                                           int act, float* scratch, void* stream) {
  return launch_n_dgrad_act(G, W, Y, gz, nullptr, M, H, N, act, scratch, stream, true);
}

TRL_API int trl_skinny_reduce_jobs(int njobs, const int* kind, const float* const* scratch, float* const* out,
                                   float* const* colsum, const int64_t* M, const int* H, const int* K,
                                   const int* out_transposed, void* stream) {
  using namespace trl;
  TRL_REQUIRE(njobs >= 0 && njobs <= kMaxRedJobs, "trl_skinny_reduce_jobs: njobs %d not in 0..%d", njobs, kMaxRedJobs);
  if (njobs == 0) return TRL_OK;
  TRL_REQUIRE(kind && scratch && out && colsum && M && H && K && out_transposed, "trl_skinny_reduce_jobs: null table");
  ReduceJobs q;
  int ctas = 0;
  for (int j = 0; j < kMaxRedJobs; ++j) {
    q.cta_begin[j] = ctas;
    if (j >= njobs) { q.partial[j] = nullptr; q.out[j] = nullptr; q.colsum[j] = nullptr; q.n_cs[j] = q.nslab[j] = q.H[j] = q.K[j] = q.out_t[j] = 0; continue; }
    TRL_REQUIRE(kind[j] >= 0 && kind[j] <= 2 && scratch[j] && M[j] >= 1 && H[j] >= 1, "trl_skinny_reduce_jobs: bad job %d", j);
    const int rows = sk_rows_per_cta(M[j]);
    q.partial[j] = scratch[j];
    q.nslab[j] = static_cast<int>(ceil_div<long long>(M[j], rows));
    q.H[j] = H[j];
    if (kind[j] == 2) {
      TRL_REQUIRE(colsum[j], "trl_skinny_reduce_jobs: job %d needs colsum", j);
      q.out[j] = colsum[j]; q.colsum[j] = colsum[j]; q.K[j] = 0; q.n_cs[j] = H[j]; q.out_t[j] = 0;
    } else {
      TRL_REQUIRE(out[j] && K[j] >= 1 && K[j] <= 24 && (kind[j] == 0 || colsum[j]), "trl_skinny_reduce_jobs: bad job %d", j);
      q.out[j] = out[j]; q.colsum[j] = colsum[j]; q.K[j] = K[j]; q.out_t[j] = out_transposed[j];
      q.n_cs[j] = colsum[j] ? (kind[j] == 1 ? H[j] : K[j]) : 0;
    }
    ctas += ceil_div(q.K[j] * q.H[j] + q.n_cs[j], kRedElems);
  }
  q.cta_begin[kMaxRedJobs] = ctas;
  q.njobs = njobs;
  skinny_reduce_jobs_kernel<<<ctas, kRedElems * kRedGroups, 0, static_cast<cudaStream_t>(stream)>>>(q);
  return check_launch("skinny_reduce_jobs_kernel");
}
```

### torchrl_b200/networks/base.py

```python
import numpy as np
import torch
import torch.nn as nn

from . import init as winit
from . import fused


class MLPBase(nn.Module):

    def __init__(self, input_shape, hidden_shapes, activation_func=nn.ReLU, init_func=winit.basic_init,
                 add_ln=False, last_activation_func=None):
        super().__init__()
        self.activation_func = activation_func
        self.add_ln = add_ln
        self.last_activation_func = last_activation_func if last_activation_func is not None else activation_func
        width = int(np.prod(input_shape))
        self.output_shape = width
        layers = []
        for i, h in enumerate(hidden_shapes):
            fc = nn.Linear(width, h)
            init_func(fc)
            layers.append(fc)
            last = (i == len(hidden_shapes) - 1)
            if last and not add_ln:
                layers.append(self.last_activation_func())
            else:
                layers.append(activation_func())
                if add_ln:
                    layers.append(nn.LayerNorm(h))
            width = h
            self.output_shape = h
        if add_ln and layers:
            layers.pop(-1)
            layers.append(self.last_activation_func())
        self.fcs = layers
        self.seq_fcs = nn.Sequential(*layers)
        self._pairs = None
        if not add_ln and len(layers) % 2 == 0 and all(isinstance(layers[i], nn.Linear) for i in range(0, len(layers), 2)):
            self._pairs = [(layers[i], layers[i + 1]) for i in range(0, len(layers), 2)]

    def forward(self, x):
        if self._pairs and fused.fused_enabled() and x.is_cuda:
            for fc, act in self._pairs:
                x = self._pair(x, fc, act)
            return x
        return self.seq_fcs(x)

    @staticmethod
    def _pair(x, fc, act):
        if fused.can_fuse(x, fc, act):
            return fused.linear_act(x, fc, fused.ACT_CODES[type(act)])
        return act(fc(x))

    def forward_with_head(self, x, head):
        if not (self._pairs and fused.fused_enabled() and x.is_cuda):
            return None
        for fc, act in self._pairs[:-1]:
            x = self._pair(x, fc, act)
        fc, act = self._pairs[-1]
        if not fused.tail_ok(x, fc, act, head):
            return head_plain(self._pair(x, fc, act), head)
        return fused.mlp_tail(x, fc, fused.ACT_CODES[type(act)], head)


def head_plain(h, head):
    if h.is_cuda and h.dtype == torch.float32:
        return fused.linear_plain(h, head)
    return head(h)


def calc_next_shape(input_shape, conv_info):
    out_channels, kernel_size, stride, padding = conv_info
    _, h, w = input_shape
    h = int((h + 2 * padding[0] - (kernel_size[0] - 1) - 1) / stride[0] + 1)
    w = int((w + 2 * padding[1] - (kernel_size[1] - 1) - 1) / stride[1] + 1)
    return (out_channels, h, w)


class CNNBase(nn.Module):

    def __init__(self, input_shape, hidden_shapes, activation_func=nn.ReLU, init_func=winit.basic_init,
                 add_ln=False, last_activation_func=None):
        super().__init__()
        self.add_ln = add_ln
        self.activation_func = activation_func
        self.last_activation_func = last_activation_func if last_activation_func is not None else activation_func
        shape = tuple(input_shape)
        channels = shape[0]
        self.output_shape = shape[0] * shape[1] * shape[2]
        layers = []
        for info in hidden_shapes:
            out_c, k, s, p = info
            conv = nn.Conv2d(channels, out_c, tuple(k), tuple(s), tuple(p))
            init_func(conv)
            layers.append(conv)
            layers.append(activation_func())
            channels = out_c
            shape = calc_next_shape(shape, info)
            if add_ln:
                layers.append(nn.LayerNorm(shape[1:]))
            self.output_shape = shape[0] * shape[1] * shape[2]
        if layers:
            layers.pop(-1)
            layers.append(self.last_activation_func())
        self.convs = layers
        self.seq_convs = nn.Sequential(*layers)

    def forward(self, x):
        lead = x.shape[:-3]
        out = self.seq_convs(x.reshape((-1,) + tuple(x.shape[-3:])))
        return out.reshape(tuple(lead) + (-1,))
```

### torchrl_b200/networks/fused.py

```python
import os
import weakref

import torch
import torch.nn as nn

from .. import _lib, ops

ACT_CODES = {nn.Tanh: 1, nn.ReLU: 2}
_ENABLED = True
_MATMUL_MODE = "tc3"
_TC3_MIN_ROWS = 2048
_TF32X3_MIN_DIM = 64
_GEMM_IMPL = os.environ.get("TORCHRL_B200_GEMM", "pair")


def set_matmul_mode(mode):
    global _MATMUL_MODE
    assert mode in ("fp32", "tf32x3", "tc3")
    _MATMUL_MODE = mode


def set_gemm_impl(impl):
    global _GEMM_IMPL
    assert impl in ("pair", "single")
    _GEMM_IMPL = impl


_FLATS = weakref.WeakSet()
_PLANES = {}
_PRESPLIT_DEPTH = 0
_TRANSPOSED = None
_T_STREAMS = {}


def _drop_planes(ptrs):
    for q in ptrs:
        _PLANES.pop(q, None)


def register_flat(flat):
    views = flat.plane_views()
    _PLANES.update(views)
    _FLATS.add(flat)
    weakref.finalize(flat, _drop_planes, list(views.keys()))


class presplit:

    def __enter__(self):
        global _PRESPLIT_DEPTH
        if _PRESPLIT_DEPTH == 0 and _MATMUL_MODE == "tc3" and _GEMM_IMPL == "pair":
            for f in list(_FLATS):
                f.refresh_split()
        _PRESPLIT_DEPTH += 1
        return self

    def __exit__(self, *a):
        global _PRESPLIT_DEPTH
        _PRESPLIT_DEPTH -= 1


def presplit_scope(fn):
    import functools

    @functools.wraps(fn)
    def wrapped(*a, **k):
        with presplit():
            return fn(*a, **k)
    return wrapped


def _planes_of(weight):
    return _PLANES.get(weight.data_ptr()) if _PRESPLIT_DEPTH > 0 else None


class transposed_planes:

    def __init__(self, *flats):
        self.flats = flats

    def __enter__(self):
        global _TRANSPOSED
        self.prev, self.event, self.joined, self.table = _TRANSPOSED, None, set(), {}
        if _PRESPLIT_DEPTH > 0 and _MATMUL_MODE == "tc3" and _GEMM_IMPL == "pair":
            self.main = torch.cuda.current_stream()
            key = self.main.cuda_stream
            if key not in _T_STREAMS:
                _T_STREAMS[key] = torch.cuda.Stream(device=self.main.device)
            self.side = _T_STREAMS[key]
            self.side.wait_stream(self.main)
            with torch.cuda.stream(self.side):
                for f in self.flats:
                    f.refresh_transposed()
                    self.table.update(f.transposed_views())
            self.event = torch.cuda.Event()
            self.event.record(self.side)
        _TRANSPOSED = self
        return self

    def __exit__(self, *a):
        global _TRANSPOSED
        _TRANSPOSED = self.prev
        if self.event is not None:
            self.main.wait_stream(self.side)

    def planes(self, weight):
        pl = self.table.get(weight.data_ptr()) if _PRESPLIT_DEPTH > 0 else None
        if pl is not None:
            st = torch.cuda.current_stream()
            if st.cuda_stream not in self.joined:
                st.wait_event(self.event)
                self.joined.add(st.cuda_stream)
        return pl


def mm_fwd(x, weight, bias=None, act=0):
    if _GEMM_IMPL == "pair":
        return ops.gemm3_pair(x, weight, planes=_planes_of(weight), bias=bias, act=act)
    return ops.gemm_tf32x3_nt(x, weight, bias=bias, act=act)


def mm_dgrad(gz, weight):
    if _GEMM_IMPL == "pair":
        planes_t = _TRANSPOSED.planes(weight) if _TRANSPOSED is not None else None
        if planes_t is not None:
            return ops.gemm3_pair(gz, weight, planes=planes_t)
        return ops.gemm3_pair(gz, weight, planes=_planes_of(weight), b_nmajor=True)
    return ops.gemm_tf32x3_nt(gz, ops.transpose_f32(weight))


def get_matmul_mode():
    return _MATMUL_MODE


def _tc3_ok(rows, n_out, k):
    return _MATMUL_MODE == "tc3" and rows >= _TC3_MIN_ROWS and n_out == 256 and k >= 32 and k % 32 == 0


def split_tf32(t):
    hi, lo = torch.empty_like(t), torch.empty_like(t)
    _lib.call("trl_split_tf32", ops._chk(t, torch.float32, "x"), t.numel(), hi.data_ptr(), lo.data_ptr(),
              ops._stream())
    return hi, lo


_WGRAD_WS = {}


def _stream_key():
    return torch.cuda.current_stream().cuda_stream


def wgrad(gz, x, out=None):
    M, H = gz.shape
    K = x.shape[1]
    if _tc3_ok(M, K, M) and H % 128 == 0 and M % (32 * 64) == 0:
        pair = _GEMM_IMPL == "pair" and H % 256 == 0
        key = (H, pair, str(gz.device), _stream_key())
        ws = _WGRAD_WS.get(key)
        if pair:
            if ws is None:
                ws = _WGRAD_WS[key] = (torch.empty(8 * H * 256, dtype=torch.float32, device=gz.device),
                                       torch.zeros(H // 8, dtype=torch.int32, device=gz.device))
            return ops.gemm3_pair_tn_cluster(gz, x, *ws, out=out, splits=64)
        if ws is None:
            ws = _WGRAD_WS[key] = torch.empty(64 * H * 256, dtype=torch.float32, device=gz.device)
        return ops.gemm_tf32x3_tn(gz, x, out=out, splits=64, workspace=ws)
    if (_MATMUL_MODE != "fp32" and K <= 24 and H % 32 == 0 and H <= 256 and _skinny_ok(gz)
            and (out is None or out.is_contiguous())):
        return skinny_tn(gz, x, out=out)
    if H < 4 or M < 4096:
        return torch.mm(gz.t(), x, out=out) if out is not None else torch.mm(gz.t(), x)
    S = 16 if min(H, K) >= 128 else 64
    while S > 1 and M % S:
        S //= 2
    if S == 1:
        return torch.mm(gz.t(), x, out=out) if out is not None else torch.mm(gz.t(), x)
    m = M // S
    part = torch.bmm(gz.view(S, m, H).transpose(1, 2), x.view(S, m, K))
    return torch.sum(part, 0, out=out) if out is not None else part.sum(0)


def mm3(a_hi, a_lo, b_hi, b_lo):
    prev = torch.backends.cuda.matmul.allow_tf32
    torch.backends.cuda.matmul.allow_tf32 = True
    try:
        out = torch.mm(a_lo, b_hi)
        out.addmm_(a_hi, b_lo)
        out.addmm_(a_hi, b_hi)
    finally:
        torch.backends.cuda.matmul.allow_tf32 = prev
    return out


_DIRECT_GRAD = False
_FORK = None
_FORK_STREAMS = {}


class backward_fork:

    def __enter__(self):
        global _FORK
        self.main = torch.cuda.current_stream()
        key = self.main.cuda_stream
        if key not in _FORK_STREAMS:
            _FORK_STREAMS[key] = torch.cuda.Stream(device=self.main.device)
        self.side = _FORK_STREAMS[key]
        self.keep, self.used, self.prev = [], False, _FORK
        _FORK = self
        return self

    def __exit__(self, *a):
        global _FORK
        _FORK = self.prev
        if self.used:
            self.main.wait_stream(self.side)
        self.keep.clear()


_FORK_ENABLED = os.environ.get("TORCHRL_B200_BWD_FORK", "1") == "1"


def _fork_here():
    f = _FORK if _FORK_ENABLED else None
    if f is not None and torch.cuda.current_stream().cuda_stream == f.main.cuda_stream:
        return f
    return None


class direct_grad:

    def __enter__(self):
        global _DIRECT_GRAD
        self.prev = _DIRECT_GRAD
        _DIRECT_GRAD = True

    def __exit__(self, *a):
        global _DIRECT_GRAD
        _DIRECT_GRAD = self.prev


def _grad_out(param):
    return param.grad if (_DIRECT_GRAD and param.grad is not None) else None


def set_fused_epilogue(flag):
    global _ENABLED
    _ENABLED = bool(flag)


def fused_enabled():
    return _ENABLED


class _Workspace:
    cache = {}

    @classmethod
    def get(cls, M, H, device):
        key = (int(M), int(H), str(device), _stream_key())
        ws = cls.cache.get(key)
        if ws is None:
            n = int(_lib.load().trl_bias_act_bwd_scratch_floats(int(M), int(H)))
            ws = (torch.empty(max(n, 4), dtype=torch.float32, device=device),
                  torch.zeros((H + 127) // 128, dtype=torch.int32, device=device))
            cls.cache[key] = ws
        return ws


_SKINNY_MIN_ROWS = 1024
_SKINNY = True
_TN_WS = {}


def set_skinny(flag):
    global _SKINNY
    _SKINNY = bool(flag)


def _skinny_ok(x):
    return _SKINNY and _ENABLED and x.is_cuda and x.shape[0] >= _SKINNY_MIN_ROWS


def _tn_scratch(M, H, K, device):
    key = (M, H, K, str(device), _stream_key())
    ws = _TN_WS.get(key)
    if ws is None:
        n = int(_lib.load().trl_skinny_tn_scratch_floats(M, H, K))
        ws = _TN_WS[key] = torch.empty(n, dtype=torch.float32, device=device)
    return ws


_DEFER = None


class deferred_reduces:
    def __enter__(self):
        global _DEFER
        self._prev = _DEFER
        _DEFER = []
        return self

    def __exit__(self, *exc):
        global _DEFER
        jobs, _DEFER = _DEFER, self._prev
        if jobs and exc[0] is None:
            raise RuntimeError("deferred_reduces: %d pending jobs; call flush_reduces() inside the scope" % len(jobs))
        return False


def _defer_scratch(kind, M, H, K, device):
    slot = len(_DEFER)
    key = ("defer", slot, kind, M, H, K, str(device))
    ws = _TN_WS.get(key)
    if ws is None:
        lib = _lib.load()
        n = int(lib.trl_skinny_dgrad_act_scratch_floats(M, H)) if kind == 2 else int(lib.trl_skinny_tn_scratch_floats(M, H, K))
        ws = _TN_WS[key] = torch.empty(n, dtype=torch.float32, device=device)
    return ws


def flush_reduces():
    import ctypes
    global _DEFER
    jobs = _DEFER
    if not jobs:
        return
    for i in range(0, len(jobs), 8):
        part = jobs[i:i + 8]
        n = len(part)
        vp = ctypes.c_void_p
        _lib.call("trl_skinny_reduce_jobs", n, (ctypes.c_int * n)(*[j[0] for j in part]),
                  (vp * n)(*[j[1].data_ptr() for j in part]),
                  (vp * n)(*[0 if j[2] is None else j[2].data_ptr() for j in part]),
                  (vp * n)(*[0 if j[3] is None else j[3].data_ptr() for j in part]),
                  (ctypes.c_int64 * n)(*[j[4] for j in part]), (ctypes.c_int * n)(*[j[5] for j in part]),
                  (ctypes.c_int * n)(*[j[6] for j in part]), (ctypes.c_int * n)(*[j[7] for j in part]), ops._stream())
    _DEFER = []


def _can_defer(*outs):
    return _DEFER is not None and all(o is not None for o in outs)


def skinny_tn(a, b, out=None, colsum=None, out_transposed=False, may_defer=False):
    M, H = a.shape
    K = b.shape[1]
    if may_defer and _can_defer(out) and len(_DEFER) < 64:
        ws = _defer_scratch(0, M, H, K, a.device)
        _lib.call("trl_skinny_tn_partial", ops._chk(a, torch.float32, "a"), ops._chk(b, torch.float32, "b"), M, H, K,
                  int(colsum is not None), ws.data_ptr(), ops._stream())
        _DEFER.append((0, ws, out, colsum, M, H, K, int(bool(out_transposed))))
        return out
    ws = _tn_scratch(M, H, K, a.device)
    if out is None:
        out = torch.empty((K, H) if out_transposed else (H, K), dtype=torch.float32, device=a.device)
    _lib.call("trl_skinny_tn", ops._chk(a, torch.float32, "a"), ops._chk(b, torch.float32, "b"),
              ops._chk(out, torch.float32, "out"), None if colsum is None else ops._chk(colsum, torch.float32, "colsum"),
              M, H, K, int(bool(out_transposed)), ws.data_ptr(), ops._stream())
    _lib.add_launches(1)
    return out


class _LinearAct(torch.autograd.Function):
    @staticmethod
    def forward(ctx, x, weight, bias, act):
        tc = (_MATMUL_MODE == "tf32x3" and min(x.shape[0], x.shape[1], weight.shape[0]) >= _TF32X3_MIN_DIM)
        if (_MATMUL_MODE != "fp32" and _skinny_ok(x) and x.shape[1] <= 24 and weight.shape[0] % 4 == 0
                and weight.shape[0] <= 1024 and weight.is_contiguous() and bias.is_contiguous()):
            z = torch.empty(x.shape[0], weight.shape[0], dtype=torch.float32, device=x.device)
            _lib.call("trl_skinny_k_fwd", x.data_ptr(), weight.data_ptr(), bias.data_ptr(), z.data_ptr(), x.shape[0],
                      x.shape[1], weight.shape[0], act, ops._stream())
            ctx.save_for_backward(x, weight, z)
            ctx.act, ctx.tc, ctx.params = act, False, (weight, bias)
            return z
        if _tc3_ok(x.shape[0], weight.shape[0], x.shape[1]) and weight.is_contiguous():
            z = mm_fwd(x, weight, bias=bias, act=act)
            ctx.save_for_backward(x, weight, z)
            ctx.act, ctx.tc, ctx.params = act, False, (weight, bias)
            return z
        elif tc:
            x_hi, x_lo = split_tf32(x)
            w_hi, w_lo = split_tf32(weight)
            z = mm3(x_hi, x_lo, w_hi.t(), w_lo.t())
            ctx.save_for_backward(x_hi, x_lo, w_hi, w_lo, z)
        else:
            z = torch.mm(x, weight.t())
            ctx.save_for_backward(x, weight, z)
        _lib.call("trl_bias_act_fwd", z.data_ptr(), ops._chk(bias, torch.float32, "bias"), z.shape[0], z.shape[1],
                  act, ops._stream())
        ctx.act = act
        ctx.tc = tc
        ctx.params = (weight, bias)
        return z

    @staticmethod
    def backward(ctx, g):
        if ctx.tc:
            return _LinearAct._backward_tc(ctx, g)
        x, weight, y = ctx.saved_tensors
        g = g if g.is_contiguous() else g.contiguous()
        M, H = y.shape
        w_param, b_param = ctx.params
        db_out, dw_out = _grad_out(b_param), _grad_out(w_param)
        db = db_out if db_out is not None else torch.empty(H, dtype=torch.float32, device=y.device)
        K = x.shape[1]
        if (not ctx.needs_input_grad[0] and _MATMUL_MODE != "fp32" and _skinny_ok(y) and K <= 24 and H % 32 == 0
                and H <= 256 and x.is_contiguous() and (dw_out is None or dw_out.is_contiguous())):
            dw = dw_out if dw_out is not None else torch.empty(H, K, dtype=torch.float32, device=y.device)
            if _can_defer(dw_out, db_out):
                ws = _defer_scratch(1, M, H, K, y.device)
                _lib.call("trl_skinny_act_wgrad_partial", g.data_ptr(), y.data_ptr(), x.data_ptr(), M, H, K, ctx.act,
                          ws.data_ptr(), ops._stream())
                _DEFER.append((1, ws, dw, db, M, H, K, 0))
                return None, None, None, None
            _lib.call("trl_skinny_act_wgrad", g.data_ptr(), y.data_ptr(), x.data_ptr(), dw.data_ptr(), db.data_ptr(),
                      M, H, K, ctx.act, _tn_scratch(M, H, K, y.device).data_ptr(), ops._stream())
            _lib.add_launches(1)
            return None, None if dw_out is not None else dw, None if db_out is not None else db, None
        gz = torch.empty_like(y)
        scratch, tickets = _Workspace.get(M, H, y.device)
        _lib.call("trl_bias_act_bwd", g.data_ptr(), y.data_ptr(), gz.data_ptr(), db.data_ptr(), M, H, ctx.act,
                  scratch.data_ptr(), tickets.data_ptr(), ops._stream())
        dx = None
        if ctx.needs_input_grad[0]:
            if _tc3_ok(M, weight.shape[1], H) and weight.is_contiguous():
                dx = mm_dgrad(gz, weight)
            else:
                dx = torch.mm(gz, weight)
        dw = wgrad(gz, x, out=dw_out) if ctx.needs_input_grad[1] else None
        return (dx, None if dw_out is not None else dw,
                None if db_out is not None else (db if ctx.needs_input_grad[2] else None), None)


def _backward_tc(ctx, g):
    x_hi, x_lo, w_hi, w_lo, y = ctx.saved_tensors
    g = g if g.is_contiguous() else g.contiguous()
    M, H = y.shape
    gz = torch.empty_like(y)
    db = torch.empty(H, dtype=torch.float32, device=y.device)
    scratch, tickets = _Workspace.get(M, H, y.device)
    _lib.call("trl_bias_act_bwd", g.data_ptr(), y.data_ptr(), gz.data_ptr(), db.data_ptr(), M, H, ctx.act,
              scratch.data_ptr(), tickets.data_ptr(), ops._stream())
    g_hi, g_lo = split_tf32(gz)
    dx = mm3(g_hi, g_lo, w_hi, w_lo) if ctx.needs_input_grad[0] else None
    dw = mm3(g_hi.t(), g_lo.t(), x_hi, x_lo) if ctx.needs_input_grad[1] else None
    return dx, dw, (db if ctx.needs_input_grad[2] else None), None


_LinearAct._backward_tc = staticmethod(_backward_tc)


class _LinearPlain(torch.autograd.Function):

    @staticmethod
    def forward(ctx, x, weight, bias):
        ctx.save_for_backward(x, weight)
        ctx.params = (weight, bias)
        N, H = weight.shape
        ctx.skinny = (_MATMUL_MODE != "fp32" and _skinny_ok(x) and N <= 8 and H in (128, 256)
                      and weight.is_contiguous())
        if ctx.skinny:
            y = torch.empty(x.shape[0], N, dtype=torch.float32, device=x.device)
            _lib.call("trl_skinny_n_fwd", x.data_ptr(), weight.data_ptr(), bias.data_ptr(), y.data_ptr(), x.shape[0], H, N,
                      ops._stream())
            return y
        return torch.addmm(bias, x, weight.t())

    @staticmethod
    def backward(ctx, g):
        x, weight = ctx.saved_tensors
        g = g if g.is_contiguous() else g.contiguous()
        w_param, b_param = ctx.params
        db_out, dw_out = _grad_out(b_param), _grad_out(w_param)
        if ctx.skinny:
            N, H = weight.shape
            dx = None
            if ctx.needs_input_grad[0]:
                dx = torch.empty(x.shape[0], H, dtype=torch.float32, device=x.device)
                _lib.call("trl_skinny_n_dgrad", g.data_ptr(), weight.data_ptr(), dx.data_ptr(), x.shape[0], H, N,
                          ops._stream())
            db = db_out if db_out is not None else torch.empty(N, dtype=torch.float32, device=x.device)
            dw = skinny_tn(x, g, out=dw_out, colsum=db, out_transposed=True)
            return dx, None if dw_out is not None else dw, None if db_out is not None else db
        dx = torch.mm(g, weight) if ctx.needs_input_grad[0] else None
        dw = wgrad(g, x, out=dw_out) if ctx.needs_input_grad[1] else None
        db = None
        if ctx.needs_input_grad[2]:
            db = torch.sum(g, 0, out=db_out) if db_out is not None else g.sum(0)
        return dx, None if dw_out is not None else dw, None if db_out is not None else db


class _MLPTail(torch.autograd.Function):

    @staticmethod
    def forward(ctx, x, w2, b2, w3, b3, act):
        y2 = mm_fwd(x, w2, bias=b2, act=act)
        M, H = y2.shape
        N = w3.shape[0]
        out = torch.empty(M, N, dtype=torch.float32, device=x.device)
        _lib.call("trl_skinny_n_fwd", y2.data_ptr(), w3.data_ptr(), b3.data_ptr(), out.data_ptr(), M, H, N,
                  ops._stream())
        ctx.save_for_backward(x, w2, y2, w3)
        ctx.act = act
        ctx.params = (w2, b2, w3, b3)
        return out

    @staticmethod
    def backward(ctx, g):
        x, w2, y2, w3 = ctx.saved_tensors
        g = g if g.is_contiguous() else g.contiguous()
        M, H = y2.shape
        N = w3.shape[0]
        dev = y2.device
        w2p, b2p, w3p, b3p = ctx.params
        dw2_out, db2_out, dw3_out, db3_out = _grad_out(w2p), _grad_out(b2p), _grad_out(w3p), _grad_out(b3p)
        db2 = db2_out if db2_out is not None else torch.empty(H, dtype=torch.float32, device=dev)
        db3 = db3_out if db3_out is not None else torch.empty(N, dtype=torch.float32, device=dev)
        gz = torch.empty_like(y2)
        if _can_defer(db2_out):
            ws = _defer_scratch(2, M, H, 0, dev)
            _lib.call("trl_skinny_n_dgrad_act_partial", g.data_ptr(), w3.data_ptr(), y2.data_ptr(), gz.data_ptr(), M, H, N,
                      ctx.act, ws.data_ptr(), ops._stream())
            _DEFER.append((2, ws, None, db2, M, H, 0, 0))
        else:
            key = ("dgrad_act", M, H, str(dev), _stream_key())
            ws = _TN_WS.get(key)
            if ws is None:
                n = int(_lib.load().trl_skinny_dgrad_act_scratch_floats(M, H))
                ws = _TN_WS[key] = torch.empty(n, dtype=torch.float32, device=dev)
            _lib.call("trl_skinny_n_dgrad_act", g.data_ptr(), w3.data_ptr(), y2.data_ptr(), gz.data_ptr(), db2.data_ptr(),
                      M, H, N, ctx.act, ws.data_ptr(), ops._stream())
            _lib.add_launches(1)
        fk = _fork_here()
        if fk is not None and dw2_out is not None and dw3_out is not None:
            fk.side.wait_stream(fk.main)
            with torch.cuda.stream(fk.side):
                dw3 = skinny_tn(y2, g, out=dw3_out, colsum=db3, out_transposed=True, may_defer=db3_out is not None)
                dw2 = wgrad(gz, x, out=dw2_out)
            fk.keep += [gz, g, y2, x]
            fk.used = True
            dx = mm_dgrad(gz, w2) if ctx.needs_input_grad[0] else None
        else:
            dw3 = skinny_tn(y2, g, out=dw3_out, colsum=db3, out_transposed=True,
                            may_defer=dw3_out is not None and db3_out is not None)
            dx = mm_dgrad(gz, w2) if ctx.needs_input_grad[0] else None
            dw2 = wgrad(gz, x, out=dw2_out)
        return (dx, None if dw2_out is not None else dw2, None if db2_out is not None else db2,
                None if dw3_out is not None else dw3, None if db3_out is not None else db3, None)


def tail_ok(h, fc, act_module, head):
    if not (_ENABLED and _SKINNY and h.is_cuda and h.dtype == torch.float32):
        return False
    rows = h.numel() // h.shape[-1]
    return (type(act_module) in ACT_CODES and rows >= max(_TC3_MIN_ROWS, _SKINNY_MIN_ROWS)
            and _tc3_ok(rows, fc.out_features, fc.in_features) and head.in_features == fc.out_features
            and head.out_features <= 8 and fc.bias is not None and head.bias is not None
            and fc.weight.is_contiguous() and head.weight.is_contiguous())


def mlp_tail(h, fc, act_code, head):
    lead = h.shape[:-1]
    h2 = h.reshape(-1, h.shape[-1])
    if not h2.is_contiguous():
        h2 = h2.contiguous()
    out = _MLPTail.apply(h2, fc.weight, fc.bias, head.weight, head.bias, act_code)
    return out.reshape(tuple(lead) + (out.shape[-1],))


def linear_plain(x, fc):
    lead = x.shape[:-1]
    x2 = x.reshape(-1, x.shape[-1])
    if not x2.is_contiguous():
        x2 = x2.contiguous()
    out = _LinearPlain.apply(x2, fc.weight, fc.bias)
    return out.reshape(tuple(lead) + (out.shape[-1],))


def linear_act(x, fc, act_code):
    lead = x.shape[:-1]
    x2 = x.reshape(-1, x.shape[-1])
    if not x2.is_contiguous():
        x2 = x2.contiguous()
    out = _LinearAct.apply(x2, fc.weight, fc.bias, act_code)
    return out.reshape(tuple(lead) + (out.shape[-1],))


def can_fuse(x, fc, act_module):
    return (_ENABLED and x.is_cuda and x.dtype == torch.float32 and type(act_module) in ACT_CODES
            and fc.out_features % 4 == 0 and fc.bias is not None)
```

### torchrl_b200/ops.py

```python
import ctypes

import torch

from . import _lib

F32, F64, U8, I32, I64 = torch.float32, torch.float64, torch.uint8, torch.int32, torch.int64


def _stream():
    return torch.cuda.current_stream().cuda_stream


class CapturedGraph:

    def __init__(self, fn):
        self.graph = torch.cuda.CUDAGraph()
        before = _lib.launch_count()
        with torch.cuda.graph(self.graph):
            fn()
        self.launches = _lib.launch_count() - before
        _lib.add_launches(-self.launches)

    def replay(self):
        self.graph.replay()
        _lib.add_launches(self.launches)


def _chk(t, dtype, name):
    if not t.is_cuda:
        raise ValueError("%s must be a CUDA tensor (torchrl_b200 has no CPU path)" % name)
    if t.dtype != dtype:
        raise TypeError("%s must be %s, got %s" % (name, dtype, t.dtype))
    if not t.is_contiguous():
        raise ValueError("%s must be contiguous" % name)
    return t.data_ptr()


def _opt(t, dtype, name):
    return None if t is None else _chk(t, dtype, name)


def _tn(t):
    if t.dim() == 3 and t.shape[2] == 1:
        return t.shape[0], t.shape[1]
    if t.dim() == 2:
        return t.shape[0], t.shape[1]
    raise ValueError("expected a (T,N) or (T,N,1) tensor, got %s" % (tuple(t.shape),))


def gae_scan(rewards, values, terminals, time_limits, last_value, gamma, tau, time_limit_filter,
             advs=None, returns=None, variant=1):
    T, N = _tn(rewards)
    if advs is None:
        advs = torch.empty_like(rewards)
    if returns is None:
        returns = torch.empty_like(rewards)
    assert values.shape == rewards.shape and terminals.shape == rewards.shape and \
        time_limits.shape == rewards.shape and last_value.numel() == N
    _lib.call("trl_gae_scan",
              _chk(rewards, F32, "rewards"), _chk(values, F32, "values"),
              _chk(terminals, U8, "terminals"), _chk(time_limits, U8, "time_limits"),
              _chk(last_value, F32, "last_value"), _chk(advs, F32, "advs"), _chk(returns, F32, "returns"),
              T, N, float(gamma), float(tau), int(bool(time_limit_filter)), int(variant), _stream())
    return advs, returns


def discount_return(rewards, values, terminals, time_limits, last_value, gamma, time_limit_filter,
                    advs=None, returns=None, variant=1):
    T, N = _tn(rewards)
    if advs is None:
        advs = torch.empty_like(rewards)
    if returns is None:
        returns = torch.empty_like(rewards)
    assert values.shape == rewards.shape and last_value.numel() == N
    _lib.call("trl_discount_return",
              _chk(rewards, F32, "rewards"), _chk(values, F32, "values"),
              _chk(terminals, U8, "terminals"), _chk(time_limits, U8, "time_limits"),
              _chk(last_value, F32, "last_value"), _chk(advs, F32, "advs"), _chk(returns, F32, "returns"),
              T, N, float(gamma), int(bool(time_limit_filter)), int(variant), _stream())
    return advs, returns


def obs_norm_moments(x, sums=None):
    N, o = x.shape
    if sums is None:
        sums = torch.empty(2 * o, dtype=F64, device=x.device)
    _lib.call("trl_obs_norm_moments", _chk(x, F32, "x"), N, o, _chk(sums, F64, "sums"), _stream())
    return sums


def obs_norm_merge(sums, batch_n, mean, var, count):
    o = mean.numel()
    _lib.call("trl_obs_norm_merge", _chk(sums, F64, "sums"), float(batch_n), o, _chk(mean, F64, "mean"),
              _chk(var, F64, "var"), _chk(count, F64, "count"), _stream())


def obs_norm_filt(raw, mean, var, clip=10.0, out=None):
    N, o = raw.shape
    if out is None:
        out = torch.empty_like(raw)
    _lib.call("trl_obs_norm_filt", _chk(raw, F32, "raw"), _chk(mean, F64, "mean"), _chk(var, F64, "var"), N, o,
              float(clip), _chk(out, F32, "out"), _stream())
    return out


def tanh_gaussian_sample(mean, log_std, eps=None, tanh_action=True, want_log_prob=False, want_pre_tanh=False,
                         want_eps=False, noise_scale=1.0, rng=None, nan_flag=None, action_out=None):
    a = mean.shape[-1]
    M = mean.numel() // a
    action = action_out if action_out is not None else torch.empty_like(mean)
    pre = torch.empty_like(mean) if want_pre_tanh else None
    logp = torch.empty(mean.shape[:-1] + (1,), dtype=F32, device=mean.device) if want_log_prob else None
    eps_out = torch.empty_like(mean) if want_eps else None
    ls_stride = 0 if log_std.dim() == 1 else a
    if ls_stride:
        assert log_std.shape == mean.shape
    seed, ctr = (0, None)
    if eps is None:
        if rng is None or rng.counter is None:
            raise ValueError("tanh_gaussian_sample needs either eps or an rng state")
        seed, ctr = rng.seed, rng.counter
    _lib.call("trl_tanh_gaussian_sample", _chk(mean, F32, "mean"), _chk(log_std, F32, "log_std"), ls_stride,
              _opt(eps, F32, "eps"), float(noise_scale), ctypes.c_uint64(seed), _opt(ctr, I64, "rng_counter"), M, a,
              int(bool(tanh_action)), _chk(action, F32, "action"), _opt(pre, F32, "pre_tanh"),
              _opt(logp, F32, "log_prob"), _opt(eps_out, F32, "eps_out"), _opt(nan_flag, I32, "nan_flag"), _stream())
    out = {"action": action}
    if pre is not None:
        out["pre_tanh"] = pre
    if logp is not None:
        out["log_prob"] = logp
    if eps_out is not None:
        out["eps"] = eps_out
    return out


def tanh_gaussian_sample_bwd(action, eps, log_std, g_action, g_logp, tanh_action):
    a = action.shape[-1]
    M = action.numel() // a
    g_mean = torch.empty_like(action)
    g_ls = torch.empty_like(action)
    ls_stride = 0 if log_std.dim() == 1 else a
    ga = g_action.contiguous() if g_action is not None else None
    gl = g_logp.contiguous() if g_logp is not None else None
    _lib.call("trl_tanh_gaussian_sample_bwd", _chk(action, F32, "action"), _chk(eps, F32, "eps"),
              _chk(log_std, F32, "log_std"), ls_stride, _opt(ga, F32, "g_action"), _opt(gl, F32, "g_logp"), M, a,
              int(bool(tanh_action)), _chk(g_mean, F32, "g_mean"), _chk(g_ls, F32, "g_log_std"), _stream())
    return g_mean, g_ls


def counter_advance(counter, t_ptr=None, T=1, size_ptr=None):
    _lib.call("trl_step_advance", _opt(t_ptr, I32, "t_ptr"), int(T), _opt(size_ptr, I32, "size_ptr"),
              _opt(counter, I64, "counter"), _stream())


class RowCopyPlan:

    def __init__(self, srcs, dsts, row_bytes):
        n = len(srcs)
        assert n == len(dsts) == len(row_bytes) and 1 <= n <= 8
        self.n = n
        self.src = (ctypes.c_void_p * n)(*[s.data_ptr() for s in srcs])
        self.dst = (ctypes.c_void_p * n)(*[d.data_ptr() for d in dsts])
        self.rb = (ctypes.c_int64 * n)(*[int(b) for b in row_bytes])
        self._keep = (list(srcs), list(dsts))


def row_bytes_of(t):
    return t[0].numel() * t.element_size()


def row_gather(plan, idx, rows, pos_ptr=None):
    _lib.call("trl_row_gather", plan.n, plan.src, plan.dst, plan.rb, _chk(idx, I64, "idx"),
              _opt(pos_ptr, I32, "pos_ptr"), int(rows), _stream())


def ring_write(plan, row_ptr):
    _lib.call("trl_ring_write", plan.n, plan.src, plan.dst, plan.rb, _chk(row_ptr, I32, "row_ptr"), _stream())


def ring_write_advance(plan, row_ptr, T, ticket, size_ptr=None):
    _lib.call("trl_ring_write_advance", plan.n, plan.src, plan.dst, plan.rb, _chk(row_ptr, I32, "row_ptr"), int(T),
              _opt(size_ptr, I32, "size_ptr"), _chk(ticket, I32, "ticket"), _stream())


def vec_stats(x, out=None):
    if out is None:
        out = torch.empty(4, dtype=F32, device=x.device)
    _lib.call("trl_vec_stats", _chk(x, F32, "x"), x.numel(), _chk(out, F32, "stats"), _stream())
    return out


class LossScratch:

    def __init__(self, B, act_dim, device, categorical=False):
        lib = _lib.load()
        n = int(lib.trl_ppo_categorical_actor_scratch_doubles(int(B)) if categorical
                else lib.trl_ppo_actor_scratch_doubles(int(B), int(act_dim)))
        self.actor = torch.zeros(max(n, 1), dtype=F64, device=device)
        self.critic = torch.zeros(max((int(B) + 255) // 256, 1), dtype=F64, device=device)
        self.tickets = torch.zeros(4, dtype=I32, device=device)
        self.B, self.a = int(B), int(act_dim)


def ppo_actor_loss(mean, log_std, actions, old_logp, advs, adv_stats, clip_para, entropy_coeff, tanh_action,
                   scratch, g_mean=None, g_log_std=None, info=None, logp_out=None, stats_pos=None, ls_clamp=None):
    ls_lo, ls_hi = (1.0, -1.0) if ls_clamp is None else (float(ls_clamp[0]), float(ls_clamp[1]))
    B, a = mean.shape
    assert scratch.B >= B and scratch.a == a
    ls_stride = 0 if log_std.dim() == 1 else a
    if g_mean is None:
        g_mean = torch.empty_like(mean)
    if g_log_std is None:
        g_log_std = torch.empty_like(log_std)
    if info is None:
        info = torch.zeros(16, dtype=F32, device=mean.device)
    _lib.call("trl_ppo_actor_loss", _chk(mean, F32, "mean"), _chk(log_std, F32, "log_std"), ls_stride,
              _chk(actions, F32, "actions"), _opt(old_logp, F32, "old_logp"), _chk(advs, F32, "advs"),
              _opt(adv_stats, F32, "adv_stats"), _opt(stats_pos, I32, "stats_pos"), B, a, int(bool(tanh_action)),
              float(clip_para),
              float(entropy_coeff), ls_lo, ls_hi, _chk(g_mean, F32, "g_mean"), _chk(g_log_std, F32, "g_log_std"),
              _opt(logp_out, F32, "logp_out"), _chk(info, F32, "info"), _chk(scratch.actor, F64, "scratch"),
              scratch.tickets[0:1].data_ptr(), _stream())
    return g_mean, g_log_std, info


def ppo_critic_loss(values, returns, old_values, clipped, clip_para, scratch, g_values=None, info=None):
    B = values.numel()
    if g_values is None:
        g_values = torch.empty_like(values)
    if info is None:
        info = torch.zeros(1, dtype=F32, device=values.device)
    _lib.call("trl_ppo_critic_loss", _chk(values, F32, "values"), _chk(returns, F32, "returns"),
              _opt(old_values, F32, "old_values"), B, int(bool(clipped)), float(clip_para),
              _chk(g_values, F32, "g_values"), _chk(info, F32, "info"), _chk(scratch.critic, F64, "scratch"),
              scratch.tickets[1:2].data_ptr(), _stream())
    return g_values, info


def gaussian_log_prob(mean, log_std, actions, tanh_action, out=None):
    B, a = mean.shape
    if out is None:
        out = torch.empty(B, dtype=F32, device=mean.device)
    ls_stride = 0 if log_std.dim() == 1 else a
    _lib.call("trl_gaussian_log_prob", _chk(mean, F32, "mean"), _chk(log_std, F32, "log_std"), ls_stride,
              _chk(actions, F32, "actions"), B, a, int(bool(tanh_action)), _chk(out, F32, "logp"), _stream())
    return out


def categorical_sample(logits, u=None, rng=None, action_out=None, want_log_prob=False, nan_flag=None):
    A = logits.shape[-1]
    M = logits.numel() // A
    action = action_out if action_out is not None else torch.empty(M, dtype=F32, device=logits.device)
    assert action.numel() == M
    logp = torch.empty(M, dtype=F32, device=logits.device) if want_log_prob else None
    seed, ctr = (0, None)
    if u is None:
        if rng is None or rng.counter is None:
            raise ValueError("categorical_sample needs either u or an rng state")
        seed, ctr = rng.seed, rng.counter
    _lib.call("trl_categorical_sample", _chk(logits, F32, "logits"), _opt(u, F32, "u"), ctypes.c_uint64(seed),
              _opt(ctr, I64, "rng_counter"), M, A, _chk(action, F32, "action"), _opt(logp, F32, "log_prob"),
              _opt(nan_flag, I32, "nan_flag"), _stream())
    return (action, logp) if want_log_prob else action


def categorical_log_prob(logits, actions, out=None):
    A = logits.shape[-1]
    M = logits.numel() // A
    if out is None:
        out = torch.empty(M, dtype=F32, device=logits.device)
    assert actions.numel() == M and out.numel() == M
    _lib.call("trl_categorical_log_prob", _chk(logits, F32, "logits"), _chk(actions, F32, "actions"), M, A,
              _chk(out, F32, "logp"), _stream())
    return out


def ppo_categorical_actor_loss(logits, actions, old_logp, advs, adv_stats, clip_para, entropy_coeff, scratch,
                               g_logits=None, info=None, logp_out=None, stats_pos=None):
    B, A = logits.shape
    assert scratch.B >= B
    if g_logits is None:
        g_logits = torch.empty_like(logits)
    if info is None:
        info = torch.zeros(16, dtype=F32, device=logits.device)
    _lib.call("trl_ppo_categorical_actor_loss", _chk(logits, F32, "logits"), _chk(actions, F32, "actions"),
              _opt(old_logp, F32, "old_logp"), _chk(advs, F32, "advs"), _opt(adv_stats, F32, "adv_stats"),
              _opt(stats_pos, I32, "stats_pos"), B, A, float(clip_para), float(entropy_coeff),
              _chk(g_logits, F32, "g_logits"), _opt(logp_out, F32, "logp_out"), _chk(info, F32, "info"),
              _chk(scratch.actor, F64, "scratch"), scratch.tickets[0:1].data_ptr(), _stream())
    return g_logits, info


def row_group_moments(x, idx, groups, b, out=None):
    n = x.numel() // x.shape[0]
    if out is None:
        out = torch.empty(groups, 4, dtype=F64, device=x.device)
    _lib.call("trl_row_group_moments", _chk(x, F32, "x"), _chk(idx, I64, "idx"), int(groups), int(b), n,
              _chk(out, F64, "moments"), _stream())
    return out


def group_stats_from_moments(gathered, world, groups, n_total, out=None):
    if out is None:
        out = torch.empty(groups, 4, dtype=F32, device=gathered.device)
    _lib.call("trl_group_stats_from_moments", _chk(gathered, F64, "moments"), int(world), int(groups), float(n_total),
              _chk(out, F32, "stats"), _stream())
    return out


def polyak_update(target_flat, source_flat, tau, planes=None):
    hi, lo = planes if planes is not None else (None, None)
    _lib.call("trl_polyak_update", _chk(target_flat, F32, "target"), _chk(source_flat, F32, "source"),
              target_flat.numel(), float(tau), _opt(hi, F32, "hi"), _opt(lo, F32, "lo"), _stream())


class OffPolicyScratch:

    def __init__(self, B, device):
        n = int(_lib.load().trl_offpolicy_scratch_doubles(int(B)))
        self.buf = [torch.zeros(max(n, 1), dtype=F64, device=device) for _ in range(5)]
        self.tickets = torch.zeros(8, dtype=I32, device=device)
        self.B = int(B)

    def t(self, i):
        return self.tickets[i:i + 1].data_ptr()


def td_target(rewards, terminals, q1_next, q2_next, logp_next, log_alpha, gamma, scratch, y=None, info=None,
              fixed_alpha=1.0):
    B = rewards.numel()
    if y is None:
        y = torch.empty(B, dtype=F32, device=rewards.device)
    if info is None:
        info = torch.zeros(1, dtype=F32, device=rewards.device)
    _lib.call("trl_td_target", _chk(rewards, F32, "rewards"), _chk(terminals, U8, "terminals"),
              _chk(q1_next, F32, "q1_next"), _opt(q2_next, F32, "q2_next"), _opt(logp_next, F32, "logp_next"),
              _opt(log_alpha, F32, "log_alpha"), float(fixed_alpha), float(gamma), B, _chk(y, F32, "y"),
              _chk(info, F32, "info"), scratch.buf[0].data_ptr(), scratch.t(0), _stream())
    return y, info


def td3_smooth_action(action, sigma, noise_clip, eps=None, rng=None, out=None):
    if out is None:
        out = torch.empty_like(action)
    seed, ctr = (0, None)
    if eps is None:
        seed, ctr = rng.seed, rng.counter
    _lib.call("trl_td3_smooth_action", _chk(action, F32, "action"), _opt(eps, F32, "eps"), float(sigma),
              float(noise_clip), ctypes.c_uint64(seed), _opt(ctr, I64, "rng_counter"), action.numel(),
              _chk(out, F32, "out"), _stream())
    return out


def sac_alpha_step(logp, target_entropy, log_alpha, adam_state, lr, scratch, info=None, betas=(0.9, 0.999), eps=1e-8):
    if info is None:
        info = torch.zeros(2, dtype=F32, device=logp.device)
    _lib.call("trl_sac_alpha_step", _chk(logp, F32, "logp"), float(target_entropy), _chk(log_alpha, F32, "log_alpha"),
              _chk(adam_state, F32, "adam_state"), float(lr), float(betas[0]), float(betas[1]), float(eps),
              logp.numel(), _chk(info, F32, "info"), scratch.buf[1].data_ptr(), scratch.t(1), _stream())
    return info


def sac_policy_loss(logp, q1, q2, log_alpha, scratch, info=None, fixed_alpha=1.0):
    B = logp.numel()
    g_lp, g1, g2 = torch.empty_like(logp), torch.empty_like(q1), torch.empty_like(q2)
    if info is None:
        info = torch.zeros(5, dtype=F32, device=logp.device)
    _lib.call("trl_sac_policy_loss", _chk(logp, F32, "logp"), _chk(q1, F32, "q1"), _chk(q2, F32, "q2"),
              _opt(log_alpha, F32, "log_alpha"), float(fixed_alpha), B, _chk(g_lp, F32, "g_logp"),
              _chk(g1, F32, "g_q1"), _chk(g2, F32, "g_q2"), _chk(info, F32, "info"), scratch.buf[2].data_ptr(),
              scratch.t(2), _stream())
    return g_lp, g1, g2, info


def twin_mse_loss(q1, q2, y, scratch, info=None):
    B = q1.numel()
    g1 = torch.empty_like(q1)
    g2 = torch.empty_like(q2) if q2 is not None else None
    if info is None:
        info = torch.zeros(2, dtype=F32, device=q1.device)
    _lib.call("trl_twin_mse_loss", _chk(q1, F32, "q1"), _opt(q2, F32, "q2"), _chk(y, F32, "y"), B,
              _chk(g1, F32, "g1"), _opt(g2, F32, "g2"), _chk(info, F32, "info"), scratch.buf[3].data_ptr(),
              scratch.t(3), _stream())
    return g1, g2, info


def qr_dqn_loss(pred, nxt, actions, rewards, terminals, gamma, scratch, n_actions, n_quantiles, mse=False, kappa=1.0,
                info=None, weights=None, td_out=None):
    B = rewards.numel()
    grad = torch.empty_like(pred)
    if info is None:
        info = torch.zeros(3, dtype=F32, device=pred.device)
    _lib.call("trl_qr_dqn_loss", _chk(pred, F32, "pred"), _chk(nxt, F32, "next"), _chk(actions, F32, "actions"),
              _chk(rewards, F32, "rewards"), _chk(terminals, U8, "terminals"), _opt(weights, F32, "weights"), B,
              int(n_actions), int(n_quantiles), float(gamma), float(kappa), int(bool(mse)), _chk(grad, F32, "grad"),
              _opt(td_out, F32, "td_out"), _chk(info, F32, "info"),
              scratch.buf[4].data_ptr(), scratch.t(4), _stream())
    return grad, info


def per_sample(prio, size, u, beta, idx=None, weights=None):
    b = u.numel()
    if idx is None:
        idx = torch.empty(b, dtype=I64, device=prio.device)
    if weights is None:
        weights = torch.empty(b, dtype=F32, device=prio.device)
    _lib.call("trl_per_sample", _chk(prio, F32, "prio"), int(size), _chk(u, F64, "u"), b, float(beta),
              _chk(idx, I64, "idx"), _chk(weights, F32, "weights"), _stream())
    return idx, weights


def per_update(prio, idx, td, alpha, eps, max_prio):
    b = idx.numel()
    n = td.numel() // b
    _lib.call("trl_per_update", _chk(prio, F32, "prio"), _chk(idx, I64, "idx"), _chk(td, F32, "td"), b, n,
              float(alpha), float(eps), _chk(max_prio, F32, "max_prio"), _stream())


def per_insert(prio, row_ptr, max_prio):
    _lib.call("trl_per_insert", _chk(prio, F32, "prio"), _chk(row_ptr, I32, "row_ptr"), _chk(max_prio, F32, "max_prio"),
              _stream())


def gemm_tf32x3_nt(a, b, out=None, splits=1, workspace=None, bias=None, act=0):
    M, K = a.shape
    assert b.shape == (256, K), "B must be (256, K)"
    if out is None:
        out = torch.empty(M, 256, dtype=F32, device=a.device)
    if splits > 1 and workspace is None:
        workspace = torch.empty(splits * M * 256, dtype=F32, device=a.device)
    _lib.call("trl_gemm_tf32x3_nt", _chk(a, F32, "a"), _chk(b, F32, "b"), _chk(out, F32, "out"), M, K, int(splits),
              None if workspace is None else workspace.data_ptr(), _opt(bias, F32, "bias"), int(act), _stream())
    if splits > 1:
        _lib.add_launches(1)
    return out


def gemm_tf32x3_tn(a, b, out=None, splits=1, workspace=None):
    K, M = a.shape
    assert b.shape == (K, 256), "B must be (K, 256)"
    if out is None:
        out = torch.empty(M, 256, dtype=F32, device=a.device)
    if splits > 1 and workspace is None:
        workspace = torch.empty(splits * M * 256, dtype=F32, device=a.device)
    _lib.call("trl_gemm_tf32x3_tn", _chk(a, F32, "a"), _chk(b, F32, "b"), _chk(out, F32, "out"), M, K, int(splits),
              None if workspace is None else workspace.data_ptr(), _stream())
    if splits > 1:
        _lib.add_launches(1)
    return out


def gemm3_pair(a, b, out=None, planes=None, b_nmajor=False, bias=None, act=0):
    M, K = a.shape
    assert tuple(b.shape) == ((K, 256) if b_nmajor else (256, K)), "B must be (K,256) if b_nmajor else (256,K)"
    if out is None:
        out = torch.empty(M, 256, dtype=F32, device=a.device)
    if planes is not None:
        hi, lo = planes
        assert hi.shape == b.shape and lo.shape == b.shape
        bh, bl = _chk(hi, F32, "b_hi"), _chk(lo, F32, "b_lo")
    else:
        bh, bl = _chk(b, F32, "b"), None
    _lib.call("trl_gemm3_pair", _chk(a, F32, "a"), bh, bl, _chk(out, F32, "out"), M, K, int(bool(b_nmajor)),
              _opt(bias, F32, "bias"), int(act), _stream())
    return out


def gemm3_pair_tn(a, b, out=None, splits=1, workspace=None):
    K, M = a.shape
    assert b.shape == (K, 256), "B must be (K, 256)"
    if out is None:
        out = torch.empty(M, 256, dtype=F32, device=a.device)
    if splits > 1 and workspace is None:
        workspace = torch.empty(splits * M * 256, dtype=F32, device=a.device)
    _lib.call("trl_gemm3_pair_tn", _chk(a, F32, "a"), _chk(b, F32, "b"), _chk(out, F32, "out"), M, K, int(splits),
              None if workspace is None else workspace.data_ptr(), _stream())
    if splits > 1:
        _lib.add_launches(1)
    return out


def gemm3_pair_tn_cluster(a, b, workspace, tickets, out=None, splits=64):
    K, M = a.shape
    assert b.shape == (K, 256), "B must be (K, 256)"
    assert workspace.numel() >= 8 * M * 256 and tickets.numel() >= M // 8, "workspace / tickets too small"
    if out is None:
        out = torch.empty(M, 256, dtype=F32, device=a.device)
    _lib.call("trl_gemm3_pair_tn_cluster", _chk(a, F32, "a"), _chk(b, F32, "b"), _chk(out, F32, "out"), M, K,
              int(splits), _chk(workspace, F32, "workspace"), _chk(tickets, torch.int32, "tickets"), _stream())
    return out


def transpose_f32(x, out=None):
    R, C = x.shape
    if out is None:
        out = torch.empty(C, R, dtype=F32, device=x.device)
    _lib.call("trl_transpose_f32", _chk(x, F32, "x"), _chk(out, F32, "out"), R, C, _stream())
    return out
```

Measured before the change: 4.700 million.

## Fuse first-layer dgrad with activation wgrad in the wgmma GEMM epilogue

Adds a wgmma GEMM variant whose epilogue takes the layer-2 dgrad tile, applies the first-layer activation derivative using a TMA-loaded Y tile, and accumulates first-layer weight and bias partials against staged input rows. The MLP tail autograd function now also absorbs the first (skinny-K) layer, so the forward runs skinny_k_fwd inline and the backward skips materializing the intermediate dgrad and the separate act_wgrad launch. This removes a full M×256 write and read plus kernel launches. In exchange the ring drops to three stages for this variant, extra shared memory and named barriers are used, and the path is limited to row counts up to a threshold.

New measurement: 4.909 million (median of 6 runs). 4.5% higher.

```diff
diff --git a/include/torchrl_b200.h b/include/torchrl_b200.h
--- a/include/torchrl_b200.h
+++ b/include/torchrl_b200.h
@@ -183,6 +183,8 @@
                       float* workspace, void* stream);
 int trl_gemm3_pair_tn_cluster(const float* A, const float* B, float* C, int64_t M, int64_t K, int splits,
                               float* workspace, int* tickets, void* stream);
+int trl_gemm3_pair_dgrad_act_wgrad(const float* G, const float* w_hi_t, const float* w_lo_t, const float* Y,
+                                   const float* X, int64_t M, int K, int act, float* scratch, void* stream);
 
 int trl_skinny_k_fwd(const float* X, const float* W, const float* bias, float* Y, int64_t M, int K, int H,
                      int act, void* stream);
diff --git a/torchrl_b200/_lib.py b/torchrl_b200/_lib.py
--- a/torchrl_b200/_lib.py
+++ b/torchrl_b200/_lib.py
@@ -83,6 +83,7 @@
     "trl_gemm3_pair": [vp, vp, vp, vp, i64, i64, i32, vp, i32, vp],
     "trl_gemm3_pair_tn": [vp, vp, vp, i64, i64, i32, vp, vp],
     "trl_gemm3_pair_tn_cluster": [vp, vp, vp, i64, i64, i32, vp, vp, vp],
+    "trl_gemm3_pair_dgrad_act_wgrad": [vp, vp, vp, vp, vp, i64, i32, i32, vp, vp],
     "trl_skinny_k_fwd": [vp, vp, vp, vp, i64, i32, i32, i32, vp],
     "trl_skinny_tn_scratch_floats": [i64, i32, i32],
     "trl_skinny_tn": [vp, vp, vp, vp, i64, i32, i32, i32, vp, vp],
diff --git a/torchrl_b200/csrc/gemm_pair_first.cu b/torchrl_b200/csrc/gemm_pair_first.cu
--- /dev/null
+++ b/torchrl_b200/csrc/gemm_pair_first.cu
@@ -0,0 +1,33 @@
+#include "gemm_wgmma.cuh"
+
+TRL_API int trl_gemm3_pair_dgrad_act_wgrad(const float* G, const float* w_hi_t, const float* w_lo_t, const float* Y,
+                                           const float* X, int64_t M, int K, int act, float* scratch, void* stream) {
+  using namespace trl;
+  using namespace trl::wg;
+  TRL_REQUIRE(M >= 1 && sk_rows_per_cta(M) <= 64, "trl_gemm3_pair_dgrad_act_wgrad: M=%lld not in [1, %d]", (long long)M,
+              64 * kSkCtas);
+  TRL_REQUIRE(K >= 1 && K <= 24, "trl_gemm3_pair_dgrad_act_wgrad: need 1<=K<=24 (K=%d)", K);
+  TRL_REQUIRE(act >= 0 && act <= 2, "trl_gemm3_pair_dgrad_act_wgrad: unknown activation %d", act);
+  TRL_REQUIRE(G && w_hi_t && w_lo_t && Y && X && scratch, "trl_gemm3_pair_dgrad_act_wgrad: null pointer");
+  TRL_REQUIRE(aligned16(G) && aligned16(w_hi_t) && aligned16(w_lo_t) && aligned16(Y) && aligned16(scratch),
+              "trl_gemm3_pair_dgrad_act_wgrad: G/W/Y/scratch must be 16-byte aligned");
+  CUtensorMap ma, mb, mb2, my;
+  if (!make_map(&ma, G, static_cast<uint64_t>(M), kN, Box::kKMajor) || !make_map(&mb, w_hi_t, kN, kN, Box::kKMajor) ||
+      !make_map(&mb2, w_lo_t, kN, kN, Box::kKMajor) || !make_map(&my, Y, static_cast<uint64_t>(M), kN, Box::kTile)) {
+    set_error("trl_gemm3_pair_dgrad_act_wgrad: cuTensorMapEncodeTiled failed");
+    return TRL_EUNSUPPORTED;
+  }
+  const int rows = sk_rows_per_cta(M);
+  Params p{nullptr, act, nullptr, M, kN / kBK, scratch, nullptr, X, rows * (64 / rows), rows};
+  cudaStream_t st = static_cast<cudaStream_t>(stream);
+  const char* what = "gemm3_wgmma_kernel<nt,split,act_wgrad>";
+#define TRL_XK(KK) \
+  case KK: return launch<false, false, true, true, false, KK>(ma, mb, mb2, p, 1, st, what, &my)
+  switch (K) {
+    TRL_XK(1); TRL_XK(2); TRL_XK(3); TRL_XK(4); TRL_XK(5); TRL_XK(6); TRL_XK(7); TRL_XK(8);
+    TRL_XK(9); TRL_XK(10); TRL_XK(11); TRL_XK(12); TRL_XK(13); TRL_XK(14); TRL_XK(15); TRL_XK(16);
+    TRL_XK(17); TRL_XK(18); TRL_XK(19); TRL_XK(20); TRL_XK(21); TRL_XK(22); TRL_XK(23); TRL_XK(24);
+  }
+#undef TRL_XK
+  return TRL_EUNSUPPORTED;
+}
diff --git a/torchrl_b200/csrc/gemm_wgmma.cuh b/torchrl_b200/csrc/gemm_wgmma.cuh
--- a/torchrl_b200/csrc/gemm_wgmma.cuh
+++ b/torchrl_b200/csrc/gemm_wgmma.cuh
@@ -1,6 +1,7 @@
 #pragma once
 #include "common.cuh"
 #include "reduce.cuh"
+#include "skinny_common.cuh"
 #include <cuda.h>
 
 namespace trl {
@@ -12,12 +13,14 @@
 constexpr int kThreads = kConsumers + 128;
 constexpr int kProducerRegs = 40, kConsumerRegs = 232;
 
-template <bool BMN, bool BSPLIT>
+template <bool BMN, bool BSPLIT, int XK = 0>
 struct Ring {
   static constexpr int kTiles = 3 + (BMN ? (BSPLIT ? 2 : 1) : 0);
   static constexpr int kStageBytes = kTiles * kTileBytes;
-  static constexpr int kStages = (200 * 1024) / kStageBytes < 4 ? (200 * 1024) / kStageBytes : 4;
-  static constexpr int kSmemBytes = kStages * kStageBytes + 1024  + 128 ;
+  static constexpr int kYBytes = XK ? kBM * kBN * 4 : 0;
+  static constexpr int kXBytes = XK ? kBM * ((XK + 3) & ~3) * 4 : 0;
+  static constexpr int kStages = XK ? 3 : ((200 * 1024) / kStageBytes < 4 ? (200 * 1024) / kStageBytes : 4);
+  static constexpr int kSmemBytes = kStages * kStageBytes + kYBytes + kXBytes + 1024  + 128 ;
   static constexpr bool kConvertB = BMN || !BSPLIT;
   static_assert(kStages >= 2 && kSmemBytes <= 227 * 1024, "fits one sm_90 CTA");
 };
@@ -157,23 +160,34 @@
   int k_blocks_per_split;
   float* __restrict__ ws;
   unsigned* tickets;
+  const float* __restrict__ X;
+  int wg_rows;
+  int slab_rows;
 };
 
 constexpr int kTileLd = kBN + 8;
 
-template <bool AMN, bool BMN, bool BSPLIT, bool TANH_MUFU, bool CLUSTER = false>
+__device__ __forceinline__ void named_sync(int id, int n) { asm volatile("bar.sync %0, %1;" ::"r"(id), "r"(n) : "memory"); }
+__device__ __forceinline__ void named_arrive(int id, int n) { asm volatile("bar.arrive %0, %1;" ::"r"(id), "r"(n) : "memory"); }
+
+template <bool AMN, bool BMN, bool BSPLIT, bool TANH_MUFU, bool CLUSTER = false, int XK = 0>
 __global__ void __launch_bounds__(kThreads, 1)
 gemm3_wgmma_kernel(const __grid_constant__ CUtensorMap map_a, const __grid_constant__ CUtensorMap map_b,
-                   const __grid_constant__ CUtensorMap map_b2, const Params p) {
-  using R = Ring<BMN, BSPLIT>;
+                   const __grid_constant__ CUtensorMap map_b2, const __grid_constant__ CUtensorMap map_y, const Params p) {
+  static_assert(XK == 0 || (!AMN && !BMN && BSPLIT && !CLUSTER), "the first-layer epilogue is a K-major pre-split dgrad");
+  using R = Ring<BMN, BSPLIT, XK>;
+  constexpr int XKP = (XK + 3) & ~3;
   constexpr int S = R::kStages;
   constexpr int kA = 0, kBhi = kTileBytes, kBlo = 2 * kTileBytes, kBraw = 3 * kTileBytes, kBraw2 = 4 * kTileBytes;
   extern __shared__ uint8_t smem_raw[];
   uint8_t* ring = reinterpret_cast<uint8_t*>((reinterpret_cast<uintptr_t>(smem_raw) + 1023) & ~static_cast<uintptr_t>(1023));
-  uint64_t* bars = reinterpret_cast<uint64_t*>(ring + S * R::kStageBytes);
+  float* ytile = reinterpret_cast<float*>(ring + S * R::kStageBytes);
+  float* xs = reinterpret_cast<float*>(ring + S * R::kStageBytes + R::kYBytes);
+  uint64_t* bars = reinterpret_cast<uint64_t*>(ring + S * R::kStageBytes + R::kYBytes + R::kXBytes);
   uint64_t* full = bars;
   uint64_t* empty = bars + S;
   uint64_t* conv = bars + 2 * S;
+  uint64_t* ybar = bars + 3 * S;
 
   const int warp = threadIdx.x >> 5, lane = threadIdx.x & 31;
   const int m_blk = blockIdx.x, n0 = blockIdx.y * kBN;
@@ -181,6 +195,7 @@
   const int split = CLUSTER ? static_cast<int>(blockIdx.z) / c_size + 8 * c_rank : static_cast<int>(blockIdx.z);
   const int nkb = p.k_blocks_per_split;
   const int kb0 = split * nkb;
+  const int m_row0 = XK ? m_blk * 2 * p.wg_rows : m_blk * kBM;
 
   if (threadIdx.x == kConsumers) {
     asm volatile("prefetch.tensormap [%0];" ::"l"(reinterpret_cast<uint64_t>(&map_a)) : "memory");
@@ -191,6 +206,7 @@
       mbar_init(&empty[s], kConsumers / 32);
       mbar_init(&conv[s], kConsumers / 32);
     }
+    if (XK) mbar_init(ybar, 1);
     asm volatile("fence.mbarrier_init.release.cluster;" ::: "memory");
   }
   __syncthreads();
@@ -209,7 +225,7 @@
 #pragma unroll
           for (int j = 0; j < 4; ++j) tma_load_2d(st + kA + j * 4096, &map_a, &full[s], m_blk * kBM + 32 * j, k0);
         } else {
-          tma_load_2d(st + kA, &map_a, &full[s], k0, m_blk * kBM);
+          tma_load_2d(st + kA, &map_a, &full[s], k0, m_row0);
         }
         if (BMN) {
           tma_load_2d(st + kBraw, &map_b, &full[s], n0, k0);
@@ -218,6 +234,18 @@
           tma_load_2d(st + kBhi, &map_b, &full[s], k0, n0);
           if (BSPLIT) tma_load_2d(st + kBlo, &map_b2, &full[s], k0, n0);
         }
+        if (XK && kb == (nkb < S ? nkb : S) - 1) {
+          mbar_arrive_expect_tx(ybar, R::kYBytes);
+          tma_load_2d(ytile, &map_y, ybar, n0, m_row0);
+        }
+      }
+    }
+    if constexpr (XK > 0) {
+      if (warp > kConsumers / 32) {
+        const long long nx = p.M - m_row0;
+        stage_rows<XK>(xs, p.X, m_row0, static_cast<int>(nx < 2 * p.wg_rows ? nx : 2 * p.wg_rows),
+                       threadIdx.x - kConsumers - 32, 96);
+        named_arrive(1, kConsumers + 96);
       }
     }
     if constexpr (CLUSTER) {
@@ -235,7 +263,7 @@
   asm volatile("setmaxnreg.inc.sync.aligned.u32 %0;" ::"n"(kConsumerRegs));
   const int ct = threadIdx.x, wgi = warp >> 2, wl = warp & 3;
   const int gid = lane >> 2, tid = lane & 3;
-  const int am = wgi * 64 + wl * 16 + gid;
+  const int am = (XK ? wgi * p.wg_rows : wgi * 64) + wl * 16 + gid;
   float acc[64], cor[64];
 #pragma unroll
   for (int i = 0; i < 64; ++i) { acc[i] = 0.f; cor[i] = 0.f; }
@@ -305,6 +333,43 @@
     if (lane == 0) mbar_arrive(&empty[s]);
   }
 
+  if constexpr (XK > 0) {
+    named_sync(2, kConsumers);
+    float* tile = reinterpret_cast<float*>(ring);
+    const int lr = wgi * 64 + wl * 16 + gid;
+#pragma unroll
+    for (int j = 0; j < 16; ++j)
+#pragma unroll
+      for (int h = 0; h < 2; ++h)
+        *reinterpret_cast<float2*>(tile + (lr + 8 * h) * kTileLd + j * 8 + 2 * tid) =
+            make_float2(acc[4 * j + 2 * h] + cor[4 * j + 2 * h], acc[4 * j + 2 * h + 1] + cor[4 * j + 2 * h + 1]);
+    named_sync(1, kConsumers + 96);
+    mbar_wait(ybar, 0);
+    const int rl = lane >> 3, cc = wl * 32 + (lane & 7) * 4;
+    const int spw = p.wg_rows / p.slab_rows;
+    const uint32_t g_u32 = smem_u32(tile + (wgi * 64) * kTileLd + cc), y_u32 = smem_u32(ytile + cc);
+    for (int sl = 0; sl < spw; ++sl) {
+      const long long slab = static_cast<long long>(m_blk * 2 + wgi) * spw + sl;
+      const long long row0 = slab * p.slab_rows;
+      if (row0 >= p.M) break;
+      const int nrows = static_cast<int>(p.M - row0 < p.slab_rows ? p.M - row0 : p.slab_rows);
+      const int gr0 = sl * p.slab_rows, br0 = wgi * p.wg_rows + sl * p.slab_rows;
+      float wacc[XKP][4];
+#pragma unroll
+      for (int k = 0; k < XKP; ++k)
+#pragma unroll
+        for (int j = 0; j < 4; ++j) wacc[k][j] = 0.f;
+      float4 asum = make_float4(0.f, 0.f, 0.f, 0.f);
+#pragma unroll 2
+      for (int r = rl; r < nrows; r += 4) {
+        const float4 g = lds128(g_u32 + static_cast<uint32_t>((gr0 + r) * kTileLd) * 4u);
+        const float4 y = lds128(y_u32 + static_cast<uint32_t>((br0 + r) * kBN) * 4u);
+        act_wgrad_row<XK>(wacc, asum, g, y, xs + (br0 + r) * XKP, p.act);
+      }
+      act_wgrad_store<XK>(p.ws + slab * (XK + 1) * kN, wacc, asum, kN, n0 + cc, rl);
+    }
+    return;
+  }
   if constexpr (CLUSTER) {
     __syncthreads();
     float* tile = reinterpret_cast<float*>(ring);
@@ -390,34 +455,36 @@
   return fn;
 }
 
-enum class Box { kKMajor, kMNMajor, kMNMajorA };
+enum class Box { kKMajor, kMNMajor, kMNMajorA, kTile };
 
 inline bool make_map(CUtensorMap* map, const float* base, uint64_t rows, uint64_t cols, Box box_kind) {
   PFN_encodeTiled enc = get_encode();
   if (!enc) return false;
   const cuuint64_t gdim[2] = {cols, rows};
   const cuuint64_t gstride[1] = {cols * sizeof(float)};
-  const cuuint32_t inner = box_kind == Box::kMNMajor ? 128 : kBK;
-  const cuuint32_t box[2] = {inner, static_cast<cuuint32_t>(box_kind == Box::kKMajor ? 128 : kBK)};
+  const bool plain = box_kind == Box::kMNMajor || box_kind == Box::kTile;
+  const cuuint32_t inner = plain ? 128 : kBK;
+  const cuuint32_t box[2] = {inner, static_cast<cuuint32_t>(box_kind == Box::kKMajor || box_kind == Box::kTile ? 128 : kBK)};
   const cuuint32_t estr[2] = {1, 1};
   return enc(map, CU_TENSOR_MAP_DATA_TYPE_FLOAT32, 2, const_cast<float*>(base), gdim, gstride, box, estr,
              CU_TENSOR_MAP_INTERLEAVE_NONE,
-             box_kind == Box::kMNMajor ? CU_TENSOR_MAP_SWIZZLE_NONE : CU_TENSOR_MAP_SWIZZLE_128B,
+             plain ? CU_TENSOR_MAP_SWIZZLE_NONE : CU_TENSOR_MAP_SWIZZLE_128B,
              CU_TENSOR_MAP_L2_PROMOTION_L2_256B, CU_TENSOR_MAP_FLOAT_OOB_FILL_NONE) == CUDA_SUCCESS;
 }
 
-template <bool AMN, bool BMN, bool BSPLIT, bool TANH_MUFU, bool CLUSTER = false>
+template <bool AMN, bool BMN, bool BSPLIT, bool TANH_MUFU, bool CLUSTER = false, int XK = 0>
 int launch(const CUtensorMap& ma, const CUtensorMap& mb, const CUtensorMap& mb2, const Params& p, unsigned splits,
-           cudaStream_t st, const char* what) {
-  constexpr int kSmem = Ring<BMN, BSPLIT>::kSmemBytes;
-  auto kernel = gemm3_wgmma_kernel<AMN, BMN, BSPLIT, TANH_MUFU, CLUSTER>;
+           cudaStream_t st, const char* what, const CUtensorMap* my = nullptr) {
+  constexpr int kSmem = Ring<BMN, BSPLIT, XK>::kSmemBytes;
+  auto kernel = gemm3_wgmma_kernel<AMN, BMN, BSPLIT, TANH_MUFU, CLUSTER, XK>;
+  const CUtensorMap& mys = my ? *my : mb2;
   static bool attr_set = false;
   if (!attr_set) {
     cudaError_t e = cudaFuncSetAttribute(kernel, cudaFuncAttributeMaxDynamicSharedMemorySize, kSmem);
     if (e != cudaSuccess) { set_error("cudaFuncSetAttribute: %s", cudaGetErrorString(e)); return static_cast<int>(e); }
     attr_set = true;
   }
-  const dim3 grid(static_cast<unsigned>(ceil_div<long long>(p.M, kBM)), kN / kBN, splits);
+  const dim3 grid(static_cast<unsigned>(ceil_div<long long>(p.M, XK ? 2 * p.wg_rows : kBM)), kN / kBN, splits);
   if constexpr (CLUSTER) {
     cudaLaunchConfig_t cfg = {};
     cfg.gridDim = grid;
@@ -431,10 +498,10 @@
     attr[0].val.clusterDim.z = splits / 8;
     cfg.attrs = attr;
     cfg.numAttrs = 1;
-    const cudaError_t e = cudaLaunchKernelEx(&cfg, kernel, ma, mb, mb2, p);
+    const cudaError_t e = cudaLaunchKernelEx(&cfg, kernel, ma, mb, mb2, mys, p);
     if (e != cudaSuccess) { set_error("%s: %s", what, cudaGetErrorString(e)); return static_cast<int>(e); }
   } else {
-    kernel<<<grid, kThreads, kSmem, st>>>(ma, mb, mb2, p);
+    kernel<<<grid, kThreads, kSmem, st>>>(ma, mb, mb2, mys, p);
   }
   return check_launch(what);
 }
diff --git a/torchrl_b200/csrc/skinny.cu b/torchrl_b200/csrc/skinny.cu
--- a/torchrl_b200/csrc/skinny.cu
+++ b/torchrl_b200/csrc/skinny.cu
@@ -1,9 +1,6 @@
-#include "common.cuh"
+#include "skinny_common.cuh"
 
 namespace trl {
-
-constexpr int kSkMaxRows = 128;
-constexpr int kSkCtas = 2 * kNumSM;
 
 __device__ __forceinline__ float sk_tanh(float x) { return tanh_ex2(x); }
 
@@ -11,39 +8,6 @@
   if (act == 1) return make_float4(sk_tanh(v.x), sk_tanh(v.y), sk_tanh(v.z), sk_tanh(v.w));
   if (act == 2) return make_float4(fmaxf(v.x, 0.f), fmaxf(v.y, 0.f), fmaxf(v.z, 0.f), fmaxf(v.w, 0.f));
   return v;
-}
-
-__device__ __forceinline__ float4 sk_dact4(float4 g, float4 y, int act) {
-  if (act == 1)
-    return make_float4(g.x * fmaf(-y.x, y.x, 1.f), g.y * fmaf(-y.y, y.y, 1.f), g.z * fmaf(-y.z, y.z, 1.f),
-                       g.w * fmaf(-y.w, y.w, 1.f));
-  if (act == 2) return make_float4(y.x > 0.f ? g.x : 0.f, y.y > 0.f ? g.y : 0.f, y.z > 0.f ? g.z : 0.f, y.w > 0.f ? g.w : 0.f);
-  return g;
-}
-
-static inline int sk_rows_per_cta(long long M) {
-  long long r = ceil_div<long long>(M, kSkCtas);
-  if (r < 8) r = 8;
-  if (r > kSkMaxRows) r = kSkMaxRows;
-  return static_cast<int>(r);
-}
-
-template <int K>
-__device__ __forceinline__ void stage_rows(float* __restrict__ dst, const float* __restrict__ src, long long row0,
-                                           int nrows, int tid, int nthr) {
-  constexpr int KP = (K + 3) & ~3;
-  const float* base = src + row0 * K;
-  for (int j = tid; j < nrows * K; j += nthr) {
-    const int r = j / K, k = j - r * K;
-    dst[r * KP + k] = __ldg(base + j);
-  }
-  if (KP != K) {
-    constexpr int PAD = KP - K > 0 ? KP - K : 1;
-    for (int j = tid; j < nrows * PAD; j += nthr) {
-      const int r = j / PAD, k = K + (j - r * PAD);
-      dst[r * KP + k] = 0.f;
-    }
-  }
 }
 
 template <int KP>
@@ -111,23 +75,6 @@
   }
 }
 
-template <int K>
-__device__ __forceinline__ void tn_fma_row(float (&acc)[(K + 3) & ~3][4], const float4 a, const float* __restrict__ brow) {
-  constexpr int KP = (K + 3) & ~3;
-  const float av[4] = {a.x, a.y, a.z, a.w};
-#pragma unroll
-  for (int q = 0; q < KP / 4; ++q) {
-    const float4 b = reinterpret_cast<const float4*>(brow)[q];
-#pragma unroll
-    for (int j = 0; j < 4; ++j) {
-      if (4 * q < K) acc[4 * q][j] = fmaf(av[j], b.x, acc[4 * q][j]);
-      if (4 * q + 1 < K) acc[4 * q + 1][j] = fmaf(av[j], b.y, acc[4 * q + 1][j]);
-      if (4 * q + 2 < K) acc[4 * q + 2][j] = fmaf(av[j], b.z, acc[4 * q + 2][j]);
-      if (4 * q + 3 < K) acc[4 * q + 3][j] = fmaf(av[j], b.w, acc[4 * q + 3][j]);
-    }
-  }
-}
-
 template <int K, bool ACT>
 __global__ void __launch_bounds__(256, 2) skinny_tn_kernel(const float* __restrict__ A, const float* __restrict__ Yact,
                                                           const float* __restrict__ B, int want_colsum, int act,
@@ -162,45 +109,24 @@
     }
 #pragma unroll
     for (int u = 0; u < U; ++u) {
-      float4 a0 = g[u];
-      if (ACT) {
-        a0 = sk_dact4(a0, y[u], act);
-        asum.x += a0.x; asum.y += a0.y; asum.z += a0.z; asum.w += a0.w;
-      }
-      tn_fma_row<K>(acc, a0, sk_smem + (r + 4 * u) * KP);
+      if (ACT) act_wgrad_row<K>(acc, asum, g[u], y[u], sk_smem + (r + 4 * u) * KP, act);
+      else tn_fma_row<K>(acc, g[u], sk_smem + (r + 4 * u) * KP);
     }
   }
   for (; r < nrows; r += 4) {
-    float4 a0 = __ldg(reinterpret_cast<const float4*>(ap + static_cast<long long>(r) * H));
-    if (ACT) {
-      a0 = sk_dact4(a0, __ldg(reinterpret_cast<const float4*>(yp + static_cast<long long>(r) * H)), act);
-      asum.x += a0.x; asum.y += a0.y; asum.z += a0.z; asum.w += a0.w;
-    }
-    tn_fma_row<K>(acc, a0, sk_smem + r * KP);
-  }
-#pragma unroll
-  for (int k = 0; k < K; ++k)
-#pragma unroll
-    for (int j = 0; j < 4; ++j) {
-      float v = acc[k][j];
-      v += __shfl_xor_sync(0xffffffffu, v, 8);
-      v += __shfl_xor_sync(0xffffffffu, v, 16);
-      acc[k][j] = v;
-    }
+    const float4 a0 = __ldg(reinterpret_cast<const float4*>(ap + static_cast<long long>(r) * H));
+    if (ACT) act_wgrad_row<K>(acc, asum, a0, __ldg(reinterpret_cast<const float4*>(yp + static_cast<long long>(r) * H)),
+                              sk_smem + r * KP, act);
+    else tn_fma_row<K>(acc, a0, sk_smem + r * KP);
+  }
   float* pp = partial + static_cast<long long>(blockIdx.x) * (K + 1) * H;
-#pragma unroll
-  for (int k = 0; k < K; ++k) {
-    if ((k & 3) == rl)
-      *reinterpret_cast<float4*>(pp + static_cast<long long>(k) * H + c0) =
-          make_float4(acc[k][0], acc[k][1], acc[k][2], acc[k][3]);
-  }
   if (ACT) {
-    asum.x += __shfl_xor_sync(0xffffffffu, asum.x, 8); asum.x += __shfl_xor_sync(0xffffffffu, asum.x, 16);
-    asum.y += __shfl_xor_sync(0xffffffffu, asum.y, 8); asum.y += __shfl_xor_sync(0xffffffffu, asum.y, 16);
-    asum.z += __shfl_xor_sync(0xffffffffu, asum.z, 8); asum.z += __shfl_xor_sync(0xffffffffu, asum.z, 16);
-    asum.w += __shfl_xor_sync(0xffffffffu, asum.w, 8); asum.w += __shfl_xor_sync(0xffffffffu, asum.w, 16);
-    if (rl == (K & 3)) *reinterpret_cast<float4*>(pp + static_cast<long long>(K) * H + c0) = asum;
-  } else if (tid < K) {
+    act_wgrad_store<K>(pp, acc, asum, H, c0, rl);
+  } else {
+    tn_combine_lanes<K>(acc);
+    tn_store_rows<K>(pp, acc, H, c0, rl);
+  }
+  if (!ACT && tid < K) {
     float s = 0.f;
     if (want_colsum)
       for (int rr = 0; rr < nrows; ++rr) s += sk_smem[rr * KP + tid];
diff --git a/torchrl_b200/csrc/skinny_common.cuh b/torchrl_b200/csrc/skinny_common.cuh
--- /dev/null
+++ b/torchrl_b200/csrc/skinny_common.cuh
@@ -0,0 +1,97 @@
+#pragma once
+#include "common.cuh"
+
+namespace trl {
+
+constexpr int kSkMaxRows = 128;
+constexpr int kSkCtas = 2 * kNumSM;
+
+static inline int sk_rows_per_cta(long long M) {
+  long long r = ceil_div<long long>(M, kSkCtas);
+  if (r < 8) r = 8;
+  if (r > kSkMaxRows) r = kSkMaxRows;
+  return static_cast<int>(r);
+}
+
+__device__ __forceinline__ float4 sk_dact4(float4 g, float4 y, int act) {
+  if (act == 1)
+    return make_float4(g.x * fmaf(-y.x, y.x, 1.f), g.y * fmaf(-y.y, y.y, 1.f), g.z * fmaf(-y.z, y.z, 1.f),
+                       g.w * fmaf(-y.w, y.w, 1.f));
+  if (act == 2) return make_float4(y.x > 0.f ? g.x : 0.f, y.y > 0.f ? g.y : 0.f, y.z > 0.f ? g.z : 0.f, y.w > 0.f ? g.w : 0.f);
+  return g;
+}
+
+template <int K>
+__device__ __forceinline__ void stage_rows(float* __restrict__ dst, const float* __restrict__ src, long long row0,
+                                           int nrows, int tid, int nthr) {
+  constexpr int KP = (K + 3) & ~3;
+  const float* base = src + row0 * K;
+  for (int j = tid; j < nrows * K; j += nthr) {
+    const int r = j / K, k = j - r * K;
+    dst[r * KP + k] = __ldg(base + j);
+  }
+  if (KP != K) {
+    constexpr int PAD = KP - K > 0 ? KP - K : 1;
+    for (int j = tid; j < nrows * PAD; j += nthr) {
+      const int r = j / PAD, k = K + (j - r * PAD);
+      dst[r * KP + k] = 0.f;
+    }
+  }
+}
+
+template <int K>
+__device__ __forceinline__ void tn_fma_row(float (&acc)[(K + 3) & ~3][4], const float4 a, const float* __restrict__ brow) {
+  constexpr int KP = (K + 3) & ~3;
+  const float av[4] = {a.x, a.y, a.z, a.w};
+#pragma unroll
+  for (int q = 0; q < KP / 4; ++q) {
+    const float4 b = reinterpret_cast<const float4*>(brow)[q];
+#pragma unroll
+    for (int j = 0; j < 4; ++j) {
+      if (4 * q < K) acc[4 * q][j] = fmaf(av[j], b.x, acc[4 * q][j]);
+      if (4 * q + 1 < K) acc[4 * q + 1][j] = fmaf(av[j], b.y, acc[4 * q + 1][j]);
+      if (4 * q + 2 < K) acc[4 * q + 2][j] = fmaf(av[j], b.z, acc[4 * q + 2][j]);
+      if (4 * q + 3 < K) acc[4 * q + 3][j] = fmaf(av[j], b.w, acc[4 * q + 3][j]);
+    }
+  }
+}
+
+template <int K>
+__device__ __forceinline__ void act_wgrad_row(float (&acc)[(K + 3) & ~3][4], float4& asum, const float4 g, const float4 y,
+                                              const float* __restrict__ xrow, int act) {
+  const float4 a0 = sk_dact4(g, y, act);
+  asum.x += a0.x; asum.y += a0.y; asum.z += a0.z; asum.w += a0.w;
+  tn_fma_row<K>(acc, a0, xrow);
+}
+
+__device__ __forceinline__ float tn_lane_sum(float v) {
+  v += __shfl_xor_sync(0xffffffffu, v, 8);
+  v += __shfl_xor_sync(0xffffffffu, v, 16);
+  return v;
+}
+template <int K>
+__device__ __forceinline__ void tn_combine_lanes(float (&acc)[(K + 3) & ~3][4]) {
+#pragma unroll
+  for (int k = 0; k < K; ++k)
+#pragma unroll
+    for (int j = 0; j < 4; ++j) acc[k][j] = tn_lane_sum(acc[k][j]);
+}
+template <int K>
+__device__ __forceinline__ void tn_store_rows(float* __restrict__ pp, const float (&acc)[(K + 3) & ~3][4], int H, int c0,
+                                              int rl) {
+#pragma unroll
+  for (int k = 0; k < K; ++k) {
+    if ((k & 3) == rl)
+      *reinterpret_cast<float4*>(pp + static_cast<long long>(k) * H + c0) = make_float4(acc[k][0], acc[k][1], acc[k][2], acc[k][3]);
+  }
+}
+template <int K>
+__device__ __forceinline__ void act_wgrad_store(float* __restrict__ pp, float (&acc)[(K + 3) & ~3][4], float4 asum, int H,
+                                                int c0, int rl) {
+  tn_combine_lanes<K>(acc);
+  tn_store_rows<K>(pp, acc, H, c0, rl);
+  asum.x = tn_lane_sum(asum.x); asum.y = tn_lane_sum(asum.y); asum.z = tn_lane_sum(asum.z); asum.w = tn_lane_sum(asum.w);
+  if (rl == (K & 3)) *reinterpret_cast<float4*>(pp + static_cast<long long>(K) * H + c0) = asum;
+}
+
+}
diff --git a/torchrl_b200/networks/base.py b/torchrl_b200/networks/base.py
--- a/torchrl_b200/networks/base.py
+++ b/torchrl_b200/networks/base.py
@@ -55,6 +55,11 @@
     def forward_with_head(self, x, head):
         if not (self._pairs and fused.fused_enabled() and x.is_cuda):
             return None
+        if len(self._pairs) == 2:
+            (fc1, act1), (fc, act) = self._pairs
+            if fused.first_ok(x, fc1, act1) and fused.tail_ok(x, fc, act, head):
+                return fused.mlp_tail(x, fc, fused.ACT_CODES[type(act)], head,
+                                      first=(fc1, fused.ACT_CODES[type(act1)]))
         for fc, act in self._pairs[:-1]:
             x = self._pair(x, fc, act)
         fc, act = self._pairs[-1]
diff --git a/torchrl_b200/networks/fused.py b/torchrl_b200/networks/fused.py
--- a/torchrl_b200/networks/fused.py
+++ b/torchrl_b200/networks/fused.py
@@ -322,22 +322,25 @@
 
 
 def flush_reduces():
-    import ctypes
     global _DEFER
     jobs = _DEFER
     if not jobs:
         return
     for i in range(0, len(jobs), 8):
-        part = jobs[i:i + 8]
-        n = len(part)
-        vp = ctypes.c_void_p
-        _lib.call("trl_skinny_reduce_jobs", n, (ctypes.c_int * n)(*[j[0] for j in part]),
-                  (vp * n)(*[j[1].data_ptr() for j in part]),
-                  (vp * n)(*[0 if j[2] is None else j[2].data_ptr() for j in part]),
-                  (vp * n)(*[0 if j[3] is None else j[3].data_ptr() for j in part]),
-                  (ctypes.c_int64 * n)(*[j[4] for j in part]), (ctypes.c_int * n)(*[j[5] for j in part]),
-                  (ctypes.c_int * n)(*[j[6] for j in part]), (ctypes.c_int * n)(*[j[7] for j in part]), ops._stream())
+        _reduce_jobs(jobs[i:i + 8])
     _DEFER = []
+
+
+def _reduce_jobs(part):
+    import ctypes
+    n = len(part)
+    vp = ctypes.c_void_p
+    _lib.call("trl_skinny_reduce_jobs", n, (ctypes.c_int * n)(*[j[0] for j in part]),
+              (vp * n)(*[j[1].data_ptr() for j in part]),
+              (vp * n)(*[0 if j[2] is None else j[2].data_ptr() for j in part]),
+              (vp * n)(*[0 if j[3] is None else j[3].data_ptr() for j in part]),
+              (ctypes.c_int64 * n)(*[j[4] for j in part]), (ctypes.c_int * n)(*[j[5] for j in part]),
+              (ctypes.c_int * n)(*[j[6] for j in part]), (ctypes.c_int * n)(*[j[7] for j in part]), ops._stream())
 
 
 def _can_defer(*outs):
@@ -367,11 +370,8 @@
     @staticmethod
     def forward(ctx, x, weight, bias, act):
         tc = (_MATMUL_MODE == "tf32x3" and min(x.shape[0], x.shape[1], weight.shape[0]) >= _TF32X3_MIN_DIM)
-        if (_MATMUL_MODE != "fp32" and _skinny_ok(x) and x.shape[1] <= 24 and weight.shape[0] % 4 == 0
-                and weight.shape[0] <= 1024 and weight.is_contiguous() and bias.is_contiguous()):
-            z = torch.empty(x.shape[0], weight.shape[0], dtype=torch.float32, device=x.device)
-            _lib.call("trl_skinny_k_fwd", x.data_ptr(), weight.data_ptr(), bias.data_ptr(), z.data_ptr(), x.shape[0],
-                      x.shape[1], weight.shape[0], act, ops._stream())
+        if _first_skinny_ok(x, weight, bias):
+            z = _skinny_first_fwd(x, weight, bias, act)
             ctx.save_for_backward(x, weight, z)
             ctx.act, ctx.tc, ctx.params = act, False, (weight, bias)
             return z
@@ -400,38 +400,59 @@
         if ctx.tc:
             return _LinearAct._backward_tc(ctx, g)
         x, weight, y = ctx.saved_tensors
-        g = g if g.is_contiguous() else g.contiguous()
-        M, H = y.shape
-        w_param, b_param = ctx.params
-        db_out, dw_out = _grad_out(b_param), _grad_out(w_param)
-        db = db_out if db_out is not None else torch.empty(H, dtype=torch.float32, device=y.device)
-        K = x.shape[1]
-        if (not ctx.needs_input_grad[0] and _MATMUL_MODE != "fp32" and _skinny_ok(y) and K <= 24 and H % 32 == 0
-                and H <= 256 and x.is_contiguous() and (dw_out is None or dw_out.is_contiguous())):
-            dw = dw_out if dw_out is not None else torch.empty(H, K, dtype=torch.float32, device=y.device)
-            if _can_defer(dw_out, db_out):
-                ws = _defer_scratch(1, M, H, K, y.device)
-                _lib.call("trl_skinny_act_wgrad_partial", g.data_ptr(), y.data_ptr(), x.data_ptr(), M, H, K, ctx.act,
-                          ws.data_ptr(), ops._stream())
-                _DEFER.append((1, ws, dw, db, M, H, K, 0))
-                return None, None, None, None
-            _lib.call("trl_skinny_act_wgrad", g.data_ptr(), y.data_ptr(), x.data_ptr(), dw.data_ptr(), db.data_ptr(),
-                      M, H, K, ctx.act, _tn_scratch(M, H, K, y.device).data_ptr(), ops._stream())
-            _lib.add_launches(1)
-            return None, None if dw_out is not None else dw, None if db_out is not None else db, None
-        gz = torch.empty_like(y)
-        scratch, tickets = _Workspace.get(M, H, y.device)
-        _lib.call("trl_bias_act_bwd", g.data_ptr(), y.data_ptr(), gz.data_ptr(), db.data_ptr(), M, H, ctx.act,
-                  scratch.data_ptr(), tickets.data_ptr(), ops._stream())
-        dx = None
-        if ctx.needs_input_grad[0]:
-            if _tc3_ok(M, weight.shape[1], H) and weight.is_contiguous():
-                dx = mm_dgrad(gz, weight)
-            else:
-                dx = torch.mm(gz, weight)
-        dw = wgrad(gz, x, out=dw_out) if ctx.needs_input_grad[1] else None
-        return (dx, None if dw_out is not None else dw,
-                None if db_out is not None else (db if ctx.needs_input_grad[2] else None), None)
+        return _linear_act_bwd(g, x, weight, y, ctx.act, ctx.params, ctx.needs_input_grad) + (None,)
+
+
+def _first_skinny_ok(x, weight, bias):
+    return (_MATMUL_MODE != "fp32" and _skinny_ok(x) and x.shape[1] <= 24 and weight.shape[0] % 4 == 0
+            and weight.shape[0] <= 1024 and weight.is_contiguous() and bias.is_contiguous())
+
+
+def _skinny_first_fwd(x, weight, bias, act):
+    z = torch.empty(x.shape[0], weight.shape[0], dtype=torch.float32, device=x.device)
+    _lib.call("trl_skinny_k_fwd", x.data_ptr(), weight.data_ptr(), bias.data_ptr(), z.data_ptr(), x.shape[0],
+              x.shape[1], weight.shape[0], act, ops._stream())
+    return z
+
+
+def _act_wgrad_ok(x, y, dw_out):
+    H = y.shape[1]
+    return (_MATMUL_MODE != "fp32" and _skinny_ok(y) and x.shape[1] <= 24 and H % 32 == 0 and H <= 256
+            and x.is_contiguous() and (dw_out is None or dw_out.is_contiguous()))
+
+
+def _linear_act_bwd(g, x, weight, y, act, params, needs_input_grad):
+    g = g if g.is_contiguous() else g.contiguous()
+    M, H = y.shape
+    w_param, b_param = params
+    db_out, dw_out = _grad_out(b_param), _grad_out(w_param)
+    db = db_out if db_out is not None else torch.empty(H, dtype=torch.float32, device=y.device)
+    K = x.shape[1]
+    if not needs_input_grad[0] and _act_wgrad_ok(x, y, dw_out):
+        dw = dw_out if dw_out is not None else torch.empty(H, K, dtype=torch.float32, device=y.device)
+        if _can_defer(dw_out, db_out):
+            ws = _defer_scratch(1, M, H, K, y.device)
+            _lib.call("trl_skinny_act_wgrad_partial", g.data_ptr(), y.data_ptr(), x.data_ptr(), M, H, K, act,
+                      ws.data_ptr(), ops._stream())
+            _DEFER.append((1, ws, dw, db, M, H, K, 0))
+            return None, None, None
+        _lib.call("trl_skinny_act_wgrad", g.data_ptr(), y.data_ptr(), x.data_ptr(), dw.data_ptr(), db.data_ptr(),
+                  M, H, K, act, _tn_scratch(M, H, K, y.device).data_ptr(), ops._stream())
+        _lib.add_launches(1)
+        return None, None if dw_out is not None else dw, None if db_out is not None else db
+    gz = torch.empty_like(y)
+    scratch, tickets = _Workspace.get(M, H, y.device)
+    _lib.call("trl_bias_act_bwd", g.data_ptr(), y.data_ptr(), gz.data_ptr(), db.data_ptr(), M, H, act,
+              scratch.data_ptr(), tickets.data_ptr(), ops._stream())
+    dx = None
+    if needs_input_grad[0]:
+        if _tc3_ok(M, weight.shape[1], H) and weight.is_contiguous():
+            dx = mm_dgrad(gz, weight)
+        else:
+            dx = torch.mm(gz, weight)
+    dw = wgrad(gz, x, out=dw_out) if needs_input_grad[1] else None
+    return (dx, None if dw_out is not None else dw,
+            None if db_out is not None else (db if needs_input_grad[2] else None))
 
 
 def _backward_tc(ctx, g):
@@ -495,26 +516,27 @@
 class _MLPTail(torch.autograd.Function):
 
     @staticmethod
-    def forward(ctx, x, w2, b2, w3, b3, act):
-        y2 = mm_fwd(x, w2, bias=b2, act=act)
+    def forward(ctx, x, w1, b1, act1, w2, b2, w3, b3, act):
+        h1 = _skinny_first_fwd(x, w1, b1, act1) if w1 is not None else x
+        y2 = mm_fwd(h1, w2, bias=b2, act=act)
         M, H = y2.shape
         N = w3.shape[0]
         out = torch.empty(M, N, dtype=torch.float32, device=x.device)
         _lib.call("trl_skinny_n_fwd", y2.data_ptr(), w3.data_ptr(), b3.data_ptr(), out.data_ptr(), M, H, N,
                   ops._stream())
-        ctx.save_for_backward(x, w2, y2, w3)
-        ctx.act = act
-        ctx.params = (w2, b2, w3, b3)
+        ctx.save_for_backward(x, w1, h1, w2, y2, w3)
+        ctx.act, ctx.act1 = act, act1
+        ctx.params = (w1, b1, w2, b2, w3, b3)
         return out
 
     @staticmethod
     def backward(ctx, g):
-        x, w2, y2, w3 = ctx.saved_tensors
+        x0, w1, x, w2, y2, w3 = ctx.saved_tensors
         g = g if g.is_contiguous() else g.contiguous()
         M, H = y2.shape
         N = w3.shape[0]
         dev = y2.device
-        w2p, b2p, w3p, b3p = ctx.params
+        w1p, b1p, w2p, b2p, w3p, b3p = ctx.params
         dw2_out, db2_out, dw3_out, db3_out = _grad_out(w2p), _grad_out(b2p), _grad_out(w3p), _grad_out(b3p)
         db2 = db2_out if db2_out is not None else torch.empty(H, dtype=torch.float32, device=dev)
         db3 = db3_out if db3_out is not None else torch.empty(N, dtype=torch.float32, device=dev)
@@ -533,6 +555,8 @@
             _lib.call("trl_skinny_n_dgrad_act", g.data_ptr(), w3.data_ptr(), y2.data_ptr(), gz.data_ptr(), db2.data_ptr(),
                       M, H, N, ctx.act, ws.data_ptr(), ops._stream())
             _lib.add_launches(1)
+        first = w1 is not None
+        want_dx = ctx.needs_input_grad[0] and not first
         fk = _fork_here()
         if fk is not None and dw2_out is not None and dw3_out is not None:
             fk.side.wait_stream(fk.main)
@@ -541,14 +565,45 @@
                 dw2 = wgrad(gz, x, out=dw2_out)
             fk.keep += [gz, g, y2, x]
             fk.used = True
-            dx = mm_dgrad(gz, w2) if ctx.needs_input_grad[0] else None
+            first_grads = _first_layer_bwd(ctx, gz, x0, w1, x, w2) if first else None
+            dx = mm_dgrad(gz, w2) if want_dx else None
         else:
             dw3 = skinny_tn(y2, g, out=dw3_out, colsum=db3, out_transposed=True,
                             may_defer=dw3_out is not None and db3_out is not None)
-            dx = mm_dgrad(gz, w2) if ctx.needs_input_grad[0] else None
+            first_grads = _first_layer_bwd(ctx, gz, x0, w1, x, w2) if first else None
+            dx = mm_dgrad(gz, w2) if want_dx else None
             dw2 = wgrad(gz, x, out=dw2_out)
-        return (dx, None if dw2_out is not None else dw2, None if db2_out is not None else db2,
+        tail = (None if dw2_out is not None else dw2, None if db2_out is not None else db2,
                 None if dw3_out is not None else dw3, None if db3_out is not None else db3, None)
+        if first:
+            return (None,) + first_grads + (None,) + tail
+        return (dx, None, None, None) + tail
+
+
+def _first_layer_bwd(ctx, gz, x0, w1, h1, w2):
+    M, H = h1.shape
+    K = x0.shape[1]
+    w1p, b1p = ctx.params[0], ctx.params[1]
+    dw_out, db_out = _grad_out(w1p), _grad_out(b1p)
+    planes_t = (_TRANSPOSED.planes(w2) if _TRANSPOSED is not None and _GEMM_IMPL == "pair" and H == 256
+                and tuple(w2.shape) == (256, 256) else None)
+    if planes_t is None or M > _DGRAD_FIRST_MAX_ROWS or not _act_wgrad_ok(x0, h1, dw_out):
+        return _linear_act_bwd(mm_dgrad(gz, w2), x0, w1, h1, ctx.act1, (w1p, b1p), (False, True, True))[1:]
+    dw = dw_out if dw_out is not None else torch.empty(H, K, dtype=torch.float32, device=h1.device)
+    db = db_out if db_out is not None else torch.empty(H, dtype=torch.float32, device=h1.device)
+    if _can_defer(dw_out, db_out):
+        ws = _defer_scratch(1, M, H, K, h1.device)
+        ops.gemm3_pair_dgrad_act_wgrad(gz, planes_t, h1, x0, ctx.act1, ws)
+        _DEFER.append((1, ws, dw, db, M, H, K, 0))
+        return None, None
+    ws = _tn_scratch(M, H, K, h1.device)
+    ops.gemm3_pair_dgrad_act_wgrad(gz, planes_t, h1, x0, ctx.act1, ws)
+    _reduce_jobs([(1, ws, dw, db, M, H, K, 0)])
+    _lib.add_launches(1)
+    return None if dw_out is not None else dw, None if db_out is not None else db
+
+
+_DGRAD_FIRST_MAX_ROWS = 16896
 
 
 def tail_ok(h, fc, act_module, head):
@@ -561,12 +616,19 @@
             and fc.weight.is_contiguous() and head.weight.is_contiguous())
 
 
-def mlp_tail(h, fc, act_code, head):
+def first_ok(x, fc, act_module):
+    if not (can_fuse(x, fc, act_module) and not x.requires_grad and x.dim() >= 1):
+        return False
+    return _first_skinny_ok(x.reshape(-1, x.shape[-1]), fc.weight, fc.bias)
+
+
+def mlp_tail(h, fc, act_code, head, first=None):
     lead = h.shape[:-1]
     h2 = h.reshape(-1, h.shape[-1])
     if not h2.is_contiguous():
         h2 = h2.contiguous()
-    out = _MLPTail.apply(h2, fc.weight, fc.bias, head.weight, head.bias, act_code)
+    w1, b1, act1 = (first[0].weight, first[0].bias, first[1]) if first is not None else (None, None, 0)
+    out = _MLPTail.apply(h2, w1, b1, act1, fc.weight, fc.bias, head.weight, head.bias, act_code)
     return out.reshape(tuple(lead) + (out.shape[-1],))
 
 
diff --git a/torchrl_b200/ops.py b/torchrl_b200/ops.py
--- a/torchrl_b200/ops.py
+++ b/torchrl_b200/ops.py
@@ -491,6 +491,15 @@
     return out
 
 
+def gemm3_pair_dgrad_act_wgrad(g, planes_t, h1, x, act, scratch):
+    M, K = x.shape
+    hi, lo = planes_t
+    assert g.shape == (M, 256) and h1.shape == (M, 256) and hi.shape == (256, 256) and lo.shape == (256, 256)
+    _lib.call("trl_gemm3_pair_dgrad_act_wgrad", _chk(g, F32, "g"), _chk(hi, F32, "w_hi_t"), _chk(lo, F32, "w_lo_t"),
+              _chk(h1, F32, "h1"), _chk(x, F32, "x"), M, K, int(act), _chk(scratch, F32, "scratch"), _stream())
+    return scratch
+
+
 def transpose_f32(x, out=None):
     R, C = x.shape
     if out is None:
```
